# jcfaracco/xpysom-dask

Hardware: AMD Instinct MI355X
Metric: samples/sec/epoch (higher is better)
Workload: dtype f16

## Files before the change

### xpysom_dask_amd/_lib.py

```python
import ctypes as C
import importlib.util
import os

HERE = os.path.dirname(os.path.abspath(__file__))
LIB_PATH = os.environ.get("SOM_LIB_PATH") or os.path.join(HERE, "libsomhip.so")

SOM_DIST = {"euclidean": 0, "euclidean_no_opt": 1, "cosine": 2, "manhattan": 3, "manhattan_no_opt": 3,
            "norm_p": 4, "norm_p_no_opt": 5}
SOM_NEIGH = {"gaussian": 0, "mexican_hat": 1, "bubble": 2, "triangle": 3}
SOM_PREC = {"f32": 0, "bf16": 1, "f16": 3, "exact": 5}
SOM_TOPO = {"rectangular": 0, "hexagonal": 1}
SOM_BMU_ACTIVATION, SOM_BMU_QUANTIZATION = 0, 1
SOM_KERNELS = {"bmu": 0, "segsum": 1, "kron": 2, "merge": 3, "prep": 4, "screen": 5}


class SomConfig(C.Structure):
    _fields_ = [("x", C.c_int32), ("y", C.c_int32), ("input_len", C.c_int32),
                ("distance", C.c_int32), ("neighborhood", C.c_int32),
                ("compact_support", C.c_int32), ("precision", C.c_int32), ("device", C.c_int32),
                ("std_coeff", C.c_double), ("stream", C.c_void_p),
                ("topology", C.c_int32), ("norm_p", C.c_int32), ("norm_p_real", C.c_double)]


_F = C.POINTER(C.c_float)
_I = C.POINTER(C.c_int32)
_H = C.c_void_p

SIGNATURES = {
    "som_version": (C.c_char_p, []),
    "som_device_count": (C.c_int, []),
    "som_last_error": (C.c_char_p, [_H]),
    "som_create": (C.c_int, [C.POINTER(SomConfig), C.POINTER(_H)]),
    "som_destroy": (None, [_H]),
    "som_set_weights": (C.c_int, [_H, _F]),
    "som_get_weights": (C.c_int, [_H, _F]),
    "som_set_data": (C.c_int, [_H, _F, C.c_int64]),
    "som_set_data_device": (C.c_int, [_H, C.c_void_p, C.c_int64]),
    "som_sync_producer": (C.c_int, [_H, C.c_uint64, C.c_int32]),
    "som_copy_to_host": (C.c_int, [_H, C.c_void_p, C.c_uint64, C.c_void_p]),
    "som_epoch_accumulate": (C.c_int, [_H, C.c_double, C.c_double, C.c_int]),
    "som_epoch_accumulate_faithful": (C.c_int, [_H, C.c_double, C.c_double, C.c_int]),
    "som_epoch_merge": (C.c_int, [_H]),
    "som_epoch": (C.c_int, [_H, C.c_double, C.c_double, C.c_int]),
    "som_epoch_accumulate_begin": (C.c_int, [_H, C.c_double, C.c_double, C.c_int]),
    "som_epoch_block_count": (C.c_int, [_H, C.POINTER(C.c_int32)]),
    "som_epoch_accumulate_block": (C.c_int, [_H, C.c_int32, C.POINTER(C.c_int64), C.POINTER(C.c_int64)]),
    "som_comm_load": (C.c_int, [C.c_char_p]),
    "som_comm_unique_id": (C.c_int, [C.c_void_p]),
    "som_comm_init": (C.c_int, [_H, C.c_int32, C.c_int32, C.c_void_p]),
    "som_epoch_allreduce": (C.c_int, [_H]),
    "som_comm_destroy": (C.c_int, [_H]),
    "som_pinned_alloc": (C.c_int, [C.c_uint64, C.POINTER(C.c_void_p)]),
    "som_pinned_free": (C.c_int, [C.c_void_p]),
    "som_stream_begin": (C.c_int, [_H]),
    "som_stream_rows": (C.c_int, [_H, _F, C.c_int64]),
    "som_stream_end": (C.c_int, [_H, C.c_double, C.c_double, C.c_int]),
    "som_accum_device_ptr": (C.c_int, [_H, C.POINTER(C.c_void_p), C.POINTER(C.c_int64)]),
    "som_get_stream": (C.c_int, [_H, C.POINTER(C.c_void_p)]),
    "som_epoch_fetch": (C.c_int, [_H, _F, _F, _I]),
    "som_epoch_accumulate_forced": (C.c_int, [_H, _I, C.c_double, C.c_double, C.c_int]),
    "som_bmu": (C.c_int, [_H, _F, C.c_int64, C.c_int32, _I]),
    "som_bmu_device": (C.c_int, [_H, C.c_void_p, C.c_int64, C.c_int32, _I]),
    "som_bmu_top2": (C.c_int, [_H, _F, C.c_int64, _I, _I]),
    "som_bmu_top2_device": (C.c_int, [_H, C.c_void_p, C.c_int64, _I, _I]),
    "som_bmu_f64": (C.c_int, [_H, C.POINTER(C.c_double), C.c_int64, _I]),
    "som_distance_matrix": (C.c_int, [_H, _F, C.c_int64, C.c_int32, _F]),
    "som_quantization_error": (C.c_int, [_H, _F, C.c_int64, C.POINTER(C.c_double)]),
    "som_quantization_error_device": (C.c_int, [_H, C.c_void_p, C.c_int64, C.POINTER(C.c_double)]),
    "som_set_verify": (C.c_int, [_H, C.c_int32]),
    "som_verify_stats": (C.c_int, [_H, C.POINTER(C.c_int64), C.POINTER(C.c_int64)]),
    "som_debug_corrupt_operands": (C.c_int, [_H, C.c_int32]),
    "som_debug_operand_crc": (C.c_int, [_H, C.c_int32, C.POINTER(C.c_uint64)]),
    "som_debug_exact_centroids": (C.c_int, [_H, C.c_int32, _F, _F, _F, _I]),
    "som_debug_mfma16": (C.c_int, [_H, C.c_void_p, C.c_void_p, _F, _F, C.c_int32]),
    "som_debug_stamps": (C.c_int, [_H, C.c_int64, C.c_void_p]),
    "som_debug_device_bytes": (C.c_int, [C.POINTER(C.c_int64)]),
    "som_debug_qe_stats": (C.c_int, [_H, C.POINTER(C.c_int64), C.POINTER(C.c_int64)]),
    "som_debug_exact_chain_stats": (C.c_int, [_H, C.POINTER(C.c_int64)]),
    "som_debug_exact_select_stats": (C.c_int, [_H, C.POINTER(C.c_int64), C.POINTER(C.c_int64), C.POINTER(C.c_int64)]),
    "som_debug_exact_plan_stats": (C.c_int, [_H, C.POINTER(C.c_int64), C.POINTER(C.c_int64)]),
    "som_debug_exact_last_plan": (C.c_int, [_H, C.POINTER(C.c_int32)]),
    "som_policy_eval": (C.c_int, [C.c_int32, C.POINTER(C.c_double), C.POINTER(C.c_double), C.POINTER(C.c_int32)]),
    "som_policy_replay": (C.c_int, [C.c_int32, C.POINTER(C.c_double), C.POINTER(C.c_double)]),
    "som_operands_replay": (C.c_int, [_I, C.c_int32, _I, _I]),
    "som_patch_order": (C.c_int, [C.c_int32, C.c_int32, _I]),
    "som_exact_stats": (C.c_int, [_H, C.POINTER(C.c_int64), C.POINTER(C.c_int64), C.POINTER(C.c_int64)]),
    "som_exact_top2_stats": (C.c_int, [_H, C.POINTER(C.c_int64), C.POINTER(C.c_int64)]),
    "som_exact_skip_stats": (C.c_int, [_H, C.POINTER(C.c_int64), C.POINTER(C.c_int64)]),
    "som_exact_resident_stats": (C.c_int, [_H, C.POINTER(C.c_int64), C.POINTER(C.c_int64)]),
    "som_exact_scout_stats": (C.c_int, [_H, C.POINTER(C.c_int64), C.POINTER(C.c_int64)]),
    "som_exact_refine_stats": (C.c_int, [_H, C.POINTER(C.c_int64), C.POINTER(C.c_int64)]),
    "som_exact_last_counts": (C.c_int, [_H, _I, C.c_int64]),
    "som_sync": (C.c_int, [_H]),
    "som_profile_enable": (C.c_int, [_H, C.c_int32]),
    "som_profile_get": (C.c_int, [_H, C.c_int32, C.POINTER(C.c_double), C.POINTER(C.c_int64)]),
    "som_profile_reset": (C.c_int, [_H]),
}

_lib = None


def torch_lib_file(name):
    try:
        spec = importlib.util.find_spec("torch")
    except (ImportError, ValueError):
        spec = None
    if spec is None or not spec.submodule_search_locations:
        return None
    cand = os.path.join(list(spec.submodule_search_locations)[0], "lib", name)
    return cand if os.path.exists(cand) else None


def _preload_torch_hip_runtime():
    try:
        spec = importlib.util.find_spec("torch")
    except (ImportError, ValueError):
        spec = None
    if spec is None or not spec.submodule_search_locations:
        return
    cand = os.path.join(list(spec.submodule_search_locations)[0], "lib", "libamdhip64.so")
    if os.path.exists(cand):
        try:
            C.CDLL(cand, mode=C.RTLD_GLOBAL)
        except OSError:
            pass


def load():
    global _lib
    if _lib is not None:
        return _lib
    if not os.path.exists(LIB_PATH):
        raise ImportError(
            f"{LIB_PATH} is missing: build it with `python -m xpysom_dask_amd.build` "
            "(needs hipcc; there is no CPU fallback)")
    if not os.environ.get("SOM_LIB_PATH"):
        from . import build as _build
        have, want = _build.built_hash(LIB_PATH), _build.source_hash()
        if have != want:
            raise ImportError(
                f"{LIB_PATH} is stale: built from sources {have}, the tree is {want}; "
                "rebuild with `python -m xpysom_dask_amd.build`")
    _preload_torch_hip_runtime()
    lib = C.CDLL(LIB_PATH)
    for name, (res, args) in SIGNATURES.items():
        fn = getattr(lib, name)
        fn.restype = res
        fn.argtypes = args
    _lib = lib
    return lib
```

### xpysom_dask_amd/csrc/exact_host.hpp

```cpp

struct PassCtr {
    int* base; int n_groups; bool whole_lines;
    int* gcount() const { return base; }
    int* gstart() const { return base + n_groups; }
    PassCounters* tail() const { return (PassCounters*)(gstart() + n_groups); }
    RowNeed* row_need() const { return (RowNeed*)base; }
    size_t bytes() const {
        const size_t b = 2 * (size_t)n_groups * sizeof(int) + sizeof(PassCounters);
        return whole_lines ? (size_t)round_up((long)b, 64) : b;
    }
};
constexpr size_t EX_CTR_TAIL_INTS = (sizeof(PassCounters) + 64) / sizeof(int);
inline PassCtr pass_ctr(const som_handle* h) { return PassCtr{h->ex.ctr, (int)cdiv(h->K, EX_GROUP), h->ex.chain}; }

constexpr double EX_KAPPA = 6.0;
ExactBound exact_bound(const som_handle* h) {
    const double u = std::ldexp(1.0, -24);
    const double Dl = h->wide ? 32.0 * h->ft_kchunks : 8.0 * h->fr_kg;
    const double n_mfma = h->wide ? h->n_kchunks : h->ks32;
    const double gamma = Dl * u / (1.0 - Dl * u);
    const double slop = 1.01;
    ExactBound eb{};
    eb.cB = (float)(slop * 2.0 * (EX_KAPPA * n_mfma + 1.0) * std::ldexp(1.0, -23));
    eb.cM = (float)(slop * 2.0);
// ... 244 lines not shown
    ex.tile_counts.reset(); ex.tlist.reset(); ex.tcnt.reset(); ex.scout_g.reset(); ex.items.reset(); ex.tile_ticket.reset();
    ex.sk_stride = 0;
    const long tiles = stride / SK_TILE;
    if (int rc = ex.sk_keys.alloc(h, (size_t)stride)) return rc;
    if (int rc = ex.sk_keys2.alloc(h, (size_t)stride)) return rc;
    if (int rc = ex.sk_vals.alloc(h, (size_t)stride)) return rc;
    if (int rc = ex.scout_g.alloc(h, (size_t)stride)) return rc;
    if (h->wide)
        if (int rc = ex.tq.alloc(h, (size_t)stride)) return rc;
    if (int rc = ex.need.alloc(h, (size_t)tiles * ex.cen[0].n_cstages)) return rc;
    if (int rc = ex.need2.alloc(h, (size_t)tiles * ex.cen[1].n_cstages)) return rc;
    if (int rc = ex.glist.alloc(h, (size_t)tiles * n_groups)) return rc;
    if (int rc = ex.gcnt.alloc(h, (size_t)tiles)) return rc;
    if (int rc = ex.tile_counts.alloc(h, (size_t)tiles)) return rc;
    if (int rc = ex.tlist.alloc(h, (size_t)tiles * n_groups * K16_T)) return rc;
    if (int rc = ex.tcnt.alloc(h, (size_t)tiles)) return rc;
    if (int rc = ex.tile_ticket.alloc(h, (size_t)tiles)) return rc;
    ex.item_slots = (int)resident_slots(h, 8);
    if (int rc = ex.items.alloc(h, (size_t)(5 * tiles + 4 * ex.item_slots + 16))) return rc;
    if (int rc = ex.sk_tmp.alloc(h, radix_scratch_ints(stride))) return rc;
    ex.sk_stride = stride;
    return 0;
}

template <class E>
int exact_skip_centroids(som_handle* h, const float* xmax2, unsigned q_blocks, unsigned long long* best64, long n_rows, bool* q_done) {
    auto& ex = h->ex;
    const float* Wsrc = h->ex_patch ? h->Wp : h->W;
    const int n_groups = (int)cdiv(h->K, EX_GROUP);
    auto& c0 = ex.cen[0];
    auto& c1 = ex.cen[1];
    const CentroidLevel l1{c0.Cc, c0.rg, c0.csq, c0.cmax2, c0.n_slots}, l2{c1.Cc, c1.rg, c1.csq, c1.cmax2, c1.n_slots};
    if (!h->ops.centroids_fresh())
        exact_centroids_kernel<<<dim3((unsigned)(cdiv(n_groups, 4) * 4)), dim3(512), 0, h->stream>>>(Wsrc, h->K, h->D, n_groups, l1, l2, h->wmax2);
    const int nst2 = ex.lp.level2 ? c1.n_cstages : 0;
    char* plain = ex.lp.scout ? c0.Cst_plain : nullptr;
    const dim3 tgrid((unsigned)cdiv((long)(c0.n_cstages + nst2) * K16_T, 4)), block(256);
    bool cm = false;
    if (h->ops.take_pending_image(&cm)) {
        const float* Wex = h->ex_patch ? h->Wp : h->W;
        float* cm1 = cm ? (float*)c0.cmax2 : nullptr;
        float* cm2 = cm ? (float*)c1.cmax2 : nullptr;
        const unsigned w_blocks = (unsigned)cdiv((long)h->n_stages * K16_T, 4);
        switch (h->ks32) {
#define SOM_PIMG_CASE(k) case k: exact_prep_images_kernel<k, E><<<dim3(w_blocks + tgrid.x + q_blocks), block, 0, h->stream>>>(w_blocks, tgrid.x, Wex, h->K, h->D, h->Wst, h->n_stages, \
            h->wmax2 + 1, h->Wst_lo, cm1, cm2, l1, c0.Cst, c0.n_cstages, l2, c1.Cst, nst2, xmax2, h->wmax2, plain, h->wn, h->stage_units, best64, n_rows); break;
        SOM_PIMG_CASE(1) SOM_PIMG_CASE(2) SOM_PIMG_CASE(3) SOM_PIMG_CASE(4)
#undef SOM_PIMG_CASE
        default: return fail(h, "exact: block skipping supports input_len <= 128");
        }
        HIPCHK(h, hipGetLastError());
        *q_done = q_blocks > 0;
        return 0;
    }
    switch (h->ks32) {
#define SOM_CIMG_CASE(k) case k: exact_centroid_image_kernel<k, E><<<tgrid, block, 0, h->stream>>>(l1, c0.Cst, c0.n_cstages, l2, c1.Cst, nst2, h->D, xmax2, h->wmax2, plain); break;
    SOM_CIMG_CASE(1) SOM_CIMG_CASE(2) SOM_CIMG_CASE(3) SOM_CIMG_CASE(4)
#undef SOM_CIMG_CASE
    default: return fail(h, "exact: block skipping supports input_len <= 128");
    }
    HIPCHK(h, hipGetLastError());
    return 0;
}

int exact_skip_sortkeys(som_handle* h, som_handle::ExactScratch::SortedRows& sr, long s0, long n, const int* prev, const int* scout_g) {
    auto& ex = h->ex;
    const int n_groups = (int)cdiv(h->K, EX_GROUP);
    if (scout_g != nullptr)
        exact_groupkey_kernel<<<dim3((unsigned)cdiv(n, 256)), dim3(256), 0, h->stream>>>(scout_g, n, n_groups, ex.sk_keys, ex.sk_vals);
    else
        exact_sortkey_kernel<<<dim3((unsigned)cdiv(n, 256)), dim3(256), 0, h->stream>>>(prev, h->ex_inv, n, h->K, ex.sk_keys, ex.sk_vals);
    int bits = 1;
    while ((1L << bits) < n_groups) ++bits;
    return radix_sort_rows(h, ex.sk_keys, n, bits, ex.sk_keys2, sr.order + s0, ex.sk_tmp);
}
template <class E>
int exact_skip_gather(som_handle* h, som_handle::ExactScratch::SortedRows& sr, long s0, const int* order, const float* X, const __bf16* Xb, long n,
                      const float* xsq, const float* xerr, const float* xmax2) {
    const long np = round_up(n, SK_TILE);
    exact_gather_sorted_kernel<E><<<dim3((unsigned)cdiv(np, 16)), dim3(256), 0, h->stream>>>(
        order, n, np, h->dp, h->D, Xb, X, xsq, xerr, xmax2, sr.Xb_s + s0 * h->dp, sr.Xl_s != nullptr ? sr.Xl_s + s0 * h->dp : nullptr, sr.Xf_s + s0 * h->D,
        sr.xsq_s + s0, sr.xerr_s + s0);
    HIPCHK(h, hipGetLastError());
    return 0;
}

template <int KS32, class E>
int exact_scout_nearest_ks(som_handle* h, const __bf16* Xb, long n, unsigned long long* best64, int* g_out) {
    auto& ex = h->ex;
    const auto& c0 = ex.cen[0];
    const void* kern = (const void*)bmu_bf16_k16_kernel<KS32, E, false, false>;
    const size_t lds = 2 * (size_t)k16_stage_bytes(KS32);
    int per_cu = 1;
    if (int rc = kernel_per_cu(h, kern, 64 * K16_NW, lds, &per_cu)) return rc;
    const long blocks = cdiv(n, K16_WG_SAMPLES);
    const long slots = resident_slots(h, per_cu);
    const int parts = std::max(1, std::min(choose_parts(h, blocks, slots, c0.n_cstages), c0.n_cstages));
    bmu_bf16_k16_kernel<KS32, E, false, false><<<dim3((unsigned)blocks, (unsigned)parts), dim3(64 * K16_NW), lds, h->stream>>>(
        Xb, n, c0.Cst_plain, c0.n_cstages, c0.n_slots, best64);
    bmu_finalize_kernel<<<dim3((unsigned)cdiv(n, 256)), dim3(256), 0, h->stream>>>(best64, n, c0.n_slots, g_out);
    HIPCHK(h, hipMemsetAsync(best64, 0xFF, (size_t)n * sizeof(unsigned long long), h->stream));
    HIPCHK(h, hipGetLastError());
    return 0;
}
template <class E>
int exact_scout_nearest(som_handle* h, const __bf16* Xb, long n, unsigned long long* best64, int* g_out) {
    SOM_KS32_DISPATCH(exact_scout_nearest_ks, h, Xb, n, best64, g_out)
    return fail(h, "exact: the scout supports input_len <= 128");
}

template <int KS32, class E>
int exact_scout_pick_ks(som_handle* h, som_handle::ExactScratch::SortedRows& sr, long s0, long n, const int* keys, unsigned long long* best64) {
    auto& ex = h->ex;
    const int n_groups = (int)cdiv(h->K, EX_GROUP);
    const long tiles = round_up(n, SK_TILE) / SK_TILE;
    const size_t lds_l = (size_t)cdiv(n_groups, 64) * sizeof(unsigned long long);
    exact_scout_lists_kernel<<<dim3((unsigned)tiles), dim3(64), lds_l, h->stream>>>(keys, nullptr, n, n_groups, ex.tlist, ex.tcnt);
    const void* kern = (const void*)bmu_bf16_k16_kernel<KS32, E, false, true>;
    const size_t lds = 2 * (size_t)k16_stage_bytes(KS32);
    int per_cu = 1;
    if (int rc = kernel_per_cu(h, kern, 64 * K16_NW, lds, &per_cu)) return rc;
    bmu_bf16_k16_kernel<KS32, E, false, true><<<dim3((unsigned)tiles, 1), dim3(64 * K16_NW), lds, h->stream>>>(
        sr.Xb_s + s0 * h->dp, n, h->Wst, h->n_stages, h->K, best64, nullptr, 0, nullptr, nullptr, nullptr, nullptr, nullptr, nullptr, ExactBound(),
        nullptr, ex.tlist, ex.tcnt);
    exact_scout_pos_kernel<<<dim3((unsigned)cdiv(n, 256)), dim3(256), 0, h->stream>>>(best64, n, h->K, sr.lastpos_s + s0);
    HIPCHK(h, hipGetLastError());
    return 0;
}
template <class E>
int exact_scout_pick(som_handle* h, som_handle::ExactScratch::SortedRows& sr, long s0, long n, const int* keys, unsigned long long* best64) {
    SOM_KS32_DISPATCH(exact_scout_pick_ks, h, sr, s0, n, keys, best64)
    return fail(h, "exact: the scout supports input_len <= 128");
}

void exact_plan_lists(som_handle* h, long tiles, int n_cstages, const unsigned long long* need2) {
    auto& ex = h->ex;
    const int n_groups = (int)cdiv(h->K, EX_GROUP);
    PassCounters* const ctr = pass_ctr(h).tail();
    const int slots = ex.item_queue ? (ex.screen_slots > 0 ? ex.screen_slots : ex.item_slots) : 0;
    int2* const queue = ex.item_queue ? ex.items + 8 : nullptr;
    int* const n_items = (int*)ex.items.p;
    if (ex.chain) {
        exact_lists_totals_kernel<<<dim3((unsigned)cdiv(tiles, LISTS_WG_TILES)), dim3(64 * LISTS_WG_TILES), 0, h->stream>>>(
            ex.need, n_cstages, need2, n_groups, ex.glist, ex.gcnt, ex.tile_counts, ex.tlist, ex.tcnt, tiles, &ctr->lists_done,
            &ctr->blocks_run, &ctr->groups_run, slots, queue, n_items, n_items + 1, ex.item_len_pct, ex.tile_ticket);
        return;
    }
    exact_lists_kernel<<<dim3((unsigned)tiles), dim3(64), 0, h->stream>>>(ex.need, n_cstages, need2, n_groups, ex.glist, ex.gcnt,
                                                                         ex.tile_counts, ex.tlist, ex.tcnt, ex.tile_ticket);
    exact_list_totals_kernel<<<dim3(1), dim3(1024), 0, h->stream>>>(ex.tile_counts, tiles, &ctr->blocks_run, &ctr->groups_run, slots, queue,
                                                                  n_items, n_items + 1, ex.item_len_pct);
}

template <int KS32, class E> constexpr bool plan_fused_fits() { return !(KS32 == 4 && std::is_same<E, Bf16>::value); }
template <class E>
int exact_skip_plan(som_handle* h, som_handle::ExactScratch::SortedRows& sr, long s0, long n, const float* xmax2, const ExactBound& eb,
                    const int* lastpos2, bool time_l2 = false) {
    auto& ex = h->ex;
    PassCounters* const ctr = pass_ctr(h).tail();
    const long np = round_up(n, SK_TILE);
    const long tiles = np / SK_TILE;
    const dim3 block(64 * K16_NW);
    const auto& c0 = ex.cen[0];
    const auto& c1 = ex.cen[1];
    const long want = (1024 + tiles - 1) / tiles;
    const long parts_cap = ex.hook_plan_parts > 0 ? ex.hook_plan_parts : 4L;
    const dim3 pgrid((unsigned)tiles, (unsigned)std::max<long>(1, std::min<long>({want, parts_cap, (long)c0.n_cstages})));
    const size_t lds1 = 2 * (size_t)h->stage_bytes + (size_t)c0.n_cstages * 8;
    const size_t lds2 = 2 * (size_t)h->stage_bytes + (size_t)c0.n_cstages * 64 * sizeof(int) + (size_t)c1.n_cstages * 8;
    const bool l2 = ex.lp.level2;
    const int force = ex.skip_mode == 3 ? 1 : 0;
    const __bf16* Xs = sr.Xb_s + s0 * h->dp;
    const size_t lds = lds2 + (size_t)c0.n_cstages * 8 + (size_t)SK_TILE * sizeof(float);
    const bool fits = h->ks32 != 4 || plan_fused_fits<4, E>();
    if (ex.fuse_plan && ex.chain && l2 && lastpos2 == nullptr && pgrid.y == 1 && !time_l2 && lds <= 160 * 1024 && fits) {
        PlanListsOut lo;
        lo.n_groups = (int)cdiv(h->K, EX_GROUP);
        lo.glist = ex.glist; lo.gcnt = ex.gcnt; lo.tile_counts = ex.tile_counts; lo.tlist = ex.tlist; lo.tcnt = ex.tcnt;
        lo.tile_ticket = ex.tile_ticket;
        lo.done = &ctr->lists_done; lo.blocks_run = &ctr->blocks_run; lo.groups_run = &ctr->groups_run;
        lo.slots = ex.item_queue ? (ex.screen_slots > 0 ? ex.screen_slots : ex.item_slots) : 0;
        lo.items = ex.item_queue ? ex.items + 8 : nullptr;
        lo.n_items = (int*)ex.items.p; lo.item_ctr = lo.n_items + 1; lo.len_pct = ex.item_len_pct;
#define SOM_PLAN_FUSED_CASE(k) case k: if constexpr (plan_fused_fits<k, E>()) { \
        { int pc; if (int rc = kernel_per_cu(h, (const void*)exact_plan_fused_kernel<k, E>, 64 * K16_NW, lds, &pc)) return rc; } \
        exact_plan_fused_kernel<k, E><<<dim3((unsigned)tiles), block, lds, h->stream>>>(Xs, n, c0.Cst, c0.n_cstages, c0.cmax2, c1.Cst, c1.n_slots, \
            c1.cmax2, sr.xsq_s + s0, sr.xerr_s + s0, xmax2, h->wmax2, h->wmax2 + 1, eb, sr.lastpos_s + s0, h->Wst, sr.seed_s + s0, force, lo); \
        } break;
        switch (h->ks32) {
        SOM_PLAN_FUSED_CASE(1) SOM_PLAN_FUSED_CASE(2) SOM_PLAN_FUSED_CASE(3) SOM_PLAN_FUSED_CASE(4)
        default: return fail(h, "exact: block skipping supports input_len <= 128");
        }
#undef SOM_PLAN_FUSED_CASE
        ++ex.plan_fused_launches;
        HIPCHK(h, hipGetLastError());
        return 0;
    }
    ++ex.plan_split_launches;
    unsigned long long* const need2_clear = l2 && ex.chain ? ex.need2.p : nullptr;
    if (l2 && !ex.chain) HIPCHK(h, hipMemsetAsync(ex.need2, 0, (size_t)tiles * c1.n_cstages * sizeof(unsigned long long), h->stream));
#define SOM_PLAN_CASE(k) case k: { \
        { int pc; if (int rc = kernel_per_cu(h, (const void*)exact_plan_kernel<k, E, false>, 64 * K16_NW, lds1, &pc)) return rc; } \
        exact_plan_kernel<k, E, false><<<pgrid, block, lds1, h->stream>>>(Xs, n, c0.Cst, c0.n_cstages, c0.rg, c0.n_slots, \
            sr.xsq_s + s0, sr.xerr_s + s0, sr.sU_s + s0, xmax2, c0.cmax2, h->wmax2, h->wmax2 + 1, eb, ex.need, sr.lastpos_s + s0, \
            h->Wst, sr.seed_s + s0, nullptr, 0, force, lastpos2, lastpos2 != nullptr ? &ctr->scout_wins : nullptr, need2_clear); \
        if (l2) { \
            if (time_l2) (void)hipEventRecord(ex.cost.ev[3], h->stream); \
            { int pc; if (int rc = kernel_per_cu(h, (const void*)exact_plan_kernel<k, E, true>, 64 * K16_NW, lds2, &pc)) return rc; } \
            exact_plan_kernel<k, E, true><<<dim3((unsigned)tiles, pgrid.y), block, lds2, h->stream>>>(Xs, n, c1.Cst, c1.n_cstages, c1.rg, c1.n_slots, \
                sr.xsq_s + s0, sr.xerr_s + s0, sr.sU_s + s0, xmax2, c1.cmax2, h->wmax2, h->wmax2 + 1, eb, ex.need2, nullptr, \
                nullptr, nullptr, ex.need, c0.n_cstages, force); \
            if (time_l2) (void)hipEventRecord(ex.cost.ev[4], h->stream); \
        } } break;
    switch (h->ks32) {
    SOM_PLAN_CASE(1) SOM_PLAN_CASE(2) SOM_PLAN_CASE(3) SOM_PLAN_CASE(4)
    default: return fail(h, "exact: block skipping supports input_len <= 128");
    }
#undef SOM_PLAN_CASE
    exact_plan_lists(h, tiles, c0.n_cstages, l2 ? ex.need2.p : nullptr);
    HIPCHK(h, hipGetLastError());
    return 0;
}

template <class E>
int exact_wide_centroids(som_handle* h, const float* xmax2) {
    auto& ex = h->ex;
    auto& c0 = ex.cen[0];
    const float* Wsrc = h->ex_patch ? h->Wp : h->W;
    const int n_groups = (int)cdiv(h->K, EX_GROUP);
    wide_centroids_kernel<<<dim3((unsigned)n_groups), dim3(256), 0, h->stream>>>(Wsrc, h->K, h->D, n_groups, c0.Cc, c0.rg, c0.csq, c0.cmax2, h->wmax2);
    const long total = (long)c0.n_img_stages * WD_T * h->n_kchunks * 64;
    prep_w_bf16_wide_kernel<E><<<dim3((unsigned)cdiv(total, 256)), dim3(256), 0, h->stream>>>(c0.Cc, n_groups, h->D, h->n_kchunks, c0.Cst, c0.n_img_stages,
                                                                                             nullptr, h->wmax2);
    exact_werr_kernel<E><<<dim3((unsigned)cdiv(n_groups, 4 * EX_WERR_UNITS)), dim3(256), 0, h->stream>>>(c0.Cc, n_groups, h->D, h->wmax2, c0.cmax2 + 1, nullptr);
    char* plain = ex.lp.scout ? c0.Cst_plain : nullptr;
    if (plain) HIPCHK(h, hipMemcpyAsync(plain, c0.Cst, (size_t)c0.n_img_stages * h->stage_bytes, hipMemcpyDeviceToDevice, h->stream));
    wide_centroid_tail_kernel<<<dim3((unsigned)cdiv((long)c0.n_img_stages * WD_STAGE_UNITS, 256)), dim3(256), 0, h->stream>>>(
        c0.rg, c0.csq, n_groups, c0.Cst, c0.n_img_stages, h->stage_bytes, xmax2, h->wmax2, plain);
    HIPCHK(h, hipGetLastError());
    return 0;
}

template <class E>
int exact_wide_gather(som_handle* h, som_handle::ExactScratch::SortedRows& sr, long s0, const float* X, long n, const float* xsq, const float* xerr,
                      const int* prev, const float* xmax2) {
    const long np = round_up(n, SK_TILE);
    wide_gather_sorted_kernel<<<dim3((unsigned)cdiv(np, 4)), dim3(256), 0, h->stream>>>(sr.order + s0, n, np, h->D, X, xsq, xerr, prev,
                                                                                      sr.Xf_s + s0 * h->D, sr.xsq_s + s0, sr.xerr_s + s0, sr.lastpos_s + s0);
    const long n_blocks = np / h->tl_bm;
    const long total = n_blocks * h->n_kchunks * (h->tl_bm / 16) * TL_KS * 64;
    prep_tiles_bf16_kernel<E><<<dim3((unsigned)cdiv(total, 256)), dim3(256), 0, h->stream>>>(
        sr.Xf_s + s0 * h->D, n, h->D, h->n_kchunks, n_blocks, h->tl_bm, h->tl_xtile, 1.0f, nullptr, (char*)(sr.Xb_s + s0 * h->dp), xmax2);
    HIPCHK(h, hipGetLastError());
    return 0;
}

template <int KS32, class E>
int exact_wide_scout_nearest_ks(som_handle* h, const __bf16* Ximg, long n, unsigned long long* best64, int* g_out) {
    auto& ex = h->ex;
    const auto& c0 = ex.cen[0];
    const size_t lds = (size_t)WD_SLOTS * wd_stage_bytes(KS32);
    int per_cu = 1;
    if (int rc = kernel_per_cu(h, (const void*)bmu_bf16_wide_kernel<KS32, E>, 64 * WD_NW, lds, &per_cu)) return rc;
    const long blocks = cdiv(n, WD_WG_SAMPLES);
    const long slots = resident_slots(h, per_cu);
    const int parts = (int)std::max<long>(1, std::min<long>({cdiv(2 * slots, blocks), 8L, (long)c0.n_img_stages}));
    bmu_bf16_wide_kernel<KS32, E><<<dim3((unsigned)blocks, (unsigned)parts), dim3(64 * WD_NW), lds, h->stream>>>(
        (const char*)Ximg, n, c0.Cst_plain, c0.n_img_stages, best64);
    bmu_finalize_kernel<<<dim3((unsigned)cdiv(n, 256)), dim3(256), 0, h->stream>>>(best64, n, c0.n_slots, g_out);
    HIPCHK(h, hipMemsetAsync(best64, 0xFF, (size_t)n * sizeof(unsigned long long), h->stream));
    HIPCHK(h, hipGetLastError());
    return 0;
}
template <int KS32, class E>
int exact_wide_scout_pick_ks(som_handle* h, som_handle::ExactScratch::SortedRows& sr, long s0, long n, const int* keys, unsigned long long* best64) {
    auto& ex = h->ex;
    const int n_groups = (int)cdiv(h->K, EX_GROUP);
    const long tiles = round_up(n, SK_TILE) / SK_TILE;
    const size_t lds_l = (size_t)cdiv(n_groups, 64) * sizeof(unsigned long long);
    exact_scout_lists_kernel<<<dim3((unsigned)tiles), dim3(64), lds_l, h->stream>>>(keys, nullptr, n, n_groups, ex.glist, ex.gcnt, 1);
    const size_t lds = (size_t)WD_SLOTS * wd_stage_bytes(KS32);
    int per_cu = 1;
    if (int rc = kernel_per_cu(h, (const void*)bmu_bf16_wide_kernel<KS32, E, false, true>, 64 * WD_NW, lds, &per_cu)) return rc;
    bmu_bf16_wide_kernel<KS32, E, false, true><<<dim3((unsigned)tiles, 1), dim3(64 * WD_NW), lds, h->stream>>>(
        (const char*)(sr.Xb_s + s0 * h->dp), n, h->Wst, h->n_stages, best64, nullptr, 0, nullptr, nullptr, nullptr, nullptr, nullptr, nullptr, ExactBound(),
        ex.glist, ex.gcnt, n_groups);
    exact_scout_pos_kernel<<<dim3((unsigned)cdiv(n, 256)), dim3(256), 0, h->stream>>>(best64, n, h->K, sr.lastpos_s + s0, h->ex_perm);
    HIPCHK(h, hipGetLastError());
    return 0;
}
template <class E>
int exact_wide_scout_nearest(som_handle* h, const __bf16* Ximg, long n, unsigned long long* best64, int* g_out) {
    SOM_WIDE_DISPATCH(exact_wide_scout_nearest_ks, h, Ximg, n, best64, g_out)
    return fail(h, "exact: no wide scout instance for this input_len");
}
template <class E>
int exact_wide_scout_pick(som_handle* h, som_handle::ExactScratch::SortedRows& sr, long s0, long n, const int* keys, unsigned long long* best64) {
    SOM_WIDE_DISPATCH(exact_wide_scout_pick_ks, h, sr, s0, n, keys, best64)
    return fail(h, "exact: no wide scout instance for this input_len");
}

template <int KS32, class E>
int exact_wide_plan_ks(som_handle* h, som_handle::ExactScratch::SortedRows& sr, long s0, long n, const float* xmax2, const ExactBound& eb) {
    auto& ex = h->ex;
    const auto& c0 = ex.cen[0];
    const long np = round_up(n, SK_TILE);
    const long tiles = np / SK_TILE;
    exact_seed_kernel<<<dim3((unsigned)cdiv(n * 16, 256)), dim3(256), 0, h->stream>>>(
        sr.Xf_s + s0 * h->D, n, h->D, h->W, h->wsq, h->K, sr.lastpos_s + s0, sr.xsq_s + s0, sr.xerr_s + s0, h->wmax2, xmax2, h->wmax2 + 1, eb, ex.seed, ex.tq);
    wide_plan_rows_kernel<<<dim3((unsigned)cdiv(n, 256)), dim3(256), 0, h->stream>>>(n, sr.xsq_s + s0, sr.xerr_s + s0, ex.tq, xmax2, c0.cmax2, h->wmax2,
                                                                                  h->wmax2 + 1, eb, ex.skip_mode == 3 ? 1 : 0, sr.seed_s + s0, sr.sU_s + s0);
    HIPCHK(h, hipMemsetAsync(ex.need, 0, (size_t)tiles * c0.n_cstages * sizeof(unsigned long long), h->stream));
    auto kern = bmu_bf16_wide_kernel<KS32, E, false, false, true>;
    const size_t lds = (size_t)WD_SLOTS * wd_stage_bytes(KS32) + (size_t)c0.n_cstages * sizeof(unsigned long long);
    int per_cu = 1;
    if (int rc = kernel_per_cu(h, (const void*)kern, 64 * WD_NW, lds, &per_cu)) return rc;
    const long slots = resident_slots(h, per_cu);
    int parts = (int)std::max<long>(1, std::min<long>({cdiv(2 * slots, tiles), 8L, (long)c0.n_img_stages}));
    bmu_bf16_wide_kernel<KS32, E, false, false, true><<<dim3((unsigned)tiles, (unsigned)parts), dim3(64 * WD_NW), lds, h->stream>>>(
        (const char*)(sr.Xb_s + s0 * h->dp), n, c0.Cst, c0.n_img_stages, nullptr, nullptr, 0, nullptr, nullptr, nullptr, nullptr, nullptr, nullptr, ExactBound(),
        nullptr, nullptr, 0, sr.seed_s + s0, sr.sU_s + s0, ex.need, c0.n_cstages);
    exact_plan_lists(h, tiles, c0.n_cstages, nullptr);
    HIPCHK(h, hipGetLastError());
    return 0;
}
template <class E>
int exact_wide_plan(som_handle* h, som_handle::ExactScratch::SortedRows& sr, long s0, long n, const float* xmax2, const ExactBound& eb) {
    SOM_WIDE_DISPATCH(exact_wide_plan_ks, h, sr, s0, n, xmax2, eb)
    return fail(h, "exact: no wide plan instance for this input_len");
}

template <int KG>
int exact_rescore_kg(som_handle* h, const float* X, unsigned long long* best64, int deint) {
    auto& ex = h->ex;
    auto kern = exact_rescore_mfma_kernel<KG>;
    const size_t lds = (size_t)fr_stage_bytes(KG);
    int per_cu = 1;
    if (int rc = kernel_per_cu(h, (const void*)kern, 256, lds, &per_cu)) return rc;
    const long grid = std::min<long>(ex.max_tiles, h->ex.grid_mult * resident_slots(h, per_cu));
    kern<<<dim3((unsigned)grid), dim3(256), lds, h->stream>>>(X, h->D, h->Wfst, h->K, ex.tile_tab, &pass_ctr(h).tail()->n_tiles, ex.plist,
                                                             best64, h->ex_perm, nullptr, h->ex_sub44 ? 1 : 0, deint, nullptr);
    return 0;
}

inline unsigned exact_tiles_blocks(const som_handle* h) { return h->ex.chain ? 16u : 1u; }

template <int KS32, class E>
int exact_refine_ks(som_handle* h, som_handle::ExactScratch::SortedRows& sr, long r0, long n, const float* xmax2, const ExactBound& eb) {
    auto& ex = h->ex;
    const PassCtr pc = pass_ctr(h);
    const int n_groups = pc.n_groups;
    int* gcount = pc.gcount(); PassCounters* const ctr = pc.tail();
    int* n_tiles = &ctr->n_tiles;
    exact_tiles_kernel<<<dim3(exact_tiles_blocks(h)), dim3(1024), 0, h->stream>>>(gcount, n_groups, ex.stride, ex.stride * ex.pairs, ex.tile_tab, n_tiles,
                                                                                 &ctr->overflow, nullptr, nullptr, &ctr->pairs_in);
    uint32_t* rowmin2 = (uint32_t*)ex.rowarg.p;
    if (!ex.chain) HIPCHK(h, hipMemsetAsync(rowmin2, 0xFF, (size_t)n * sizeof(uint32_t), h->stream));
    const size_t lds = (size_t)k16_stage_bytes(KS32) + (size_t)K16_T * KS32 * 1024;
    int per_cu = 1;
    if (int rc = kernel_per_cu(h, (const void*)exact_refine_kernel<KS32, E>, 256, lds, &per_cu)) return rc;
    const long grid = std::min<long>(ex.max_tiles, h->ex.grid_mult * resident_slots(h, per_cu));
    exact_refine_kernel<KS32, E><<<dim3((unsigned)grid), dim3(256), lds, h->stream>>>(
        sr.Xb_s + r0 * h->dp, sr.Xl_s + r0 * h->dp, h->Wst, h->Wst_lo, ex.tile_tab, n_tiles, ex.plist, ex.gmin, rowmin2);
    exact_thr2_kernel<<<dim3((unsigned)cdiv(n, 256)), dim3(256), 0, h->stream>>>(rowmin2, n, sr.xsq_s + r0, sr.xerr_s + r0, h->wmax2, xmax2,
                                                                               h->wmax2 + 1, eb);
    exact_select2_kernel<<<dim3((unsigned)n_groups), dim3(256), 0, h->stream>>>(ex.plist, ex.gmin, ex.stride, gcount, rowmin2, &ctr->pairs_out);
    HIPCHK(h, hipGetLastError());
    return 0;
}
template <class E>
int exact_refine(som_handle* h, som_handle::ExactScratch::SortedRows& sr, long r0, long n, const float* xmax2, const ExactBound& eb) {
// ... 365 lines not shown
```

### xpysom_dask_amd/csrc/exact_skip.hpp

```cpp
#pragma once
#include "bmu_bf16_k16.hpp"
#include "bmu_f32_res.hpp"

namespace somhip {

constexpr int SK_TILE = K16_WG_SAMPLES;
static_assert(K16_STAGE_UNITS == 64 && K16_T == 4, "block skipping: a stage of the resident screen is one 64-unit group of four 16-unit tiles");

struct CentroidLevel { float* C; float* rg; float* csq; float* cmax2; int n_slots; };
struct CentroidShared {
    float qsum[4][128];
    float part[2][64][2];
    float csq_s[2][5];
};
__device__ __forceinline__ void group_centroids(const float (&w)[16], int g, int K, int D, const CentroidLevel& l1,
                                                const CentroidLevel& l2, CentroidShared& sh) {
    const int tid = threadIdx.x, lane = tid & 63;
    const int d = tid & 127, q = tid >> 7, fh = (tid >> 6) & 1;
    const int cnt = (int)max(0L, min(64L, (long)K - (long)g * 64));
    const int cb = max(0, min(16, cnt - 16 * q));
    float sum = 0.0f;
#pragma unroll
    for (int k = 0; k < 16; ++k) sum += w[k];
    sh.qsum[q][d] = sum;
// ... 67 lines not shown
    __shared__ int u_s[64];
    __shared__ float den_s[64];
    const int g = blockIdx.x, tid = threadIdx.x;
    const int d = tid & 127, q = tid >> 7;
    const int cnt = (int)max(0L, min(64L, (long)K - (long)g * 64));
    const int cb = max(0, min(16, cnt - 16 * q));
    if (tid < cnt) {
        const int pos = g * 64 + tid;
        const int u = o.perm != nullptr ? o.perm[pos] : pos;
        u_s[tid] = u;
        den_s[tid] = ACC[(long)u * D1p + D];
    }
    __syncthreads();
    float w[16];
#pragma unroll
    for (int k = 0; k < 16; ++k) {
        const bool on = d < D && k < cb;
        const long u = on ? u_s[16 * q + k] : 0;
        const float* src = !on ? ACC : den_s[16 * q + k] != 0.0f ? ACC + u * D1p + d : o.W + u * D + d;
        const float v = *src;
        w[k] = on ? v : 0.0f;
    }
#pragma unroll
    for (int k = 0; k < 16; ++k) {
        const bool on = d < D && k < cb;
        const int i = 16 * q + k;
        const float den = on ? den_s[i] : 0.0f;
        const float v = w[k] / den;
        w[k] = den != 0.0f ? v : w[k];
        if (on) {
            const long u = u_s[i];
            if (den != 0.0f) o.W[u * D + d] = w[k];
            if (o.Wp != nullptr) o.Wp[((long)g * 64 + i) * D + d] = w[k];
            ws[i * MPX_STRIDE + d] = w[k];
        }
    }
    if (l1.C != nullptr && g == 0 && tid == 0) { l1.cmax2[1] = 0.0f; l2.cmax2[1] = 0.0f; }
    if (l1.C != nullptr) group_centroids(w, g, K, D, l1, l2, sh);
    else __syncthreads();
    if (g >= n_groups) return;
    if (o.Wfst != nullptr) {
        char* base = o.Wfst + (long)g * fr_stage_bytes(o.fr_kg);
        for (int r = tid; r < FR_UT * o.fr_kg * 64; r += 512) {
            const int lane = r & 63, t = r >> 6;
            const int gk = t % o.fr_kg, i = (t / o.fr_kg) * 32 + (lane & 31);
            f32x4 v;
#pragma unroll
            for (int j = 0; j < 4; ++j) {
                const int k = 8 * gk + 2 * j + (lane >> 5);
                v[j] = (i < cnt && k < D) ? ws[i * MPX_STRIDE + k] : 0.0f;
            }
            *(f32x4*)(base + (long)r * 16) = v;
        }
    }
    if (tid < 64) {
        float qv = __builtin_inff(), m = 0.0f;
        if (tid < cnt) {
            const int pos = g * 64 + tid;
            qv = np_pairwise_sq_sum_leaf((const float*)(ws + tid * MPX_STRIDE), D);
            o.wsq[u_s[tid]] = qv;
            if (o.wsq_p != nullptr) o.wsq_p[pos] = qv;
            o.wn[pos] = qv;
            m = (qv == qv) ? qv : 0.0f;
        }
        if (o.Wfst != nullptr) ((float*)(o.Wfst + (long)g * fr_stage_bytes(o.fr_kg) + (long)FR_UT * o.fr_kg * 1024))[tid] = qv;
#pragma unroll
        for (int s = 32; s > 0; s >>= 1) m = fmaxf(m, __shfl_xor(m, s, 64));
        if (tid == 0) atomic_max_pos_f32(o.wmax2, m);
    }
}

__global__ __launch_bounds__(256) void exact_sortkey_kernel(const int* __restrict__ prev, const int* __restrict__ inv, long n,
                                                            int K, int* __restrict__ keys, int* __restrict__ vals) {
    const long i = (long)blockIdx.x * 256 + threadIdx.x;
    if (i >= n) return;
    int u = prev[i];
    u = u < 0 ? 0 : u >= K ? K - 1 : u;
    keys[i] = (inv != nullptr ? inv[u] : u) >> 6;
    vals[i] = (int)i;
}

__global__ __launch_bounds__(256) void exact_lastpos_kernel(const int* __restrict__ prev, const int* __restrict__ order,
                                                            const int* __restrict__ inv, long n, int K, int* __restrict__ lastpos) {
    const long p = (long)blockIdx.x * 256 + threadIdx.x;
    if (p >= n) return;
    int u = prev[order[p]];
    u = u < 0 ? 0 : u >= K ? K - 1 : u;
    lastpos[p] = inv != nullptr ? inv[u] : u;
}

template <class EL>
__global__ __launch_bounds__(256) void exact_gather_sorted_kernel(const int* __restrict__ order, long n, long np, int dp, int D,
                                                                  const __bf16* __restrict__ Xb, const float* __restrict__ X,
                                                                  const float* __restrict__ xsq, const float* __restrict__ xerr,
                                                                  const float* __restrict__ xmax2,
                                                                  __bf16* __restrict__ Xb_s, __bf16* __restrict__ Xl_s,
                                                                  float* __restrict__ Xf_s,
                                                                  float* __restrict__ xsq_s, float* __restrict__ xerr_s) {
    using E = typename EL::T;
    using bf16x8 = typename V8<E>::t;
    const int lane = threadIdx.x & 15;
    const long p = (long)blockIdx.x * 16 + (threadIdx.x >> 4);
    if (p >= np) return;
    const long r = p < n ? (long)order[p] : -1;
    const float sx = ex_scale(*xmax2);
    const bool vec = (D & 7) == 0;
    for (int c = lane; c < dp / 8; c += 16) {
        bf16x8 v, vl;
#pragma unroll
        for (int j = 0; j < 8; ++j) { v[j] = (E)0.0f; vl[j] = (E)0.0f; }
        if (r >= 0) {
            v = *(const bf16x8*)((const char*)Xb + (r * dp + c * 8) * 2);
            float f[8];
            if (vec && c * 8 < D) {
                const f32x4 a = *(const f32x4*)(X + r * D + c * 8), b = *(const f32x4*)(X + r * D + c * 8 + 4);
                const f32x4 ev = {a[0], a[2], b[0], b[2]}, od = {a[1], a[3], b[1], b[3]};
                *(f32x4*)(Xf_s + p * D + c * 4) = ev;
                *(f32x4*)(Xf_s + p * D + D / 2 + c * 4) = od;
#pragma unroll
                for (int j = 0; j < 4; ++j) { f[j] = a[j]; f[4 + j] = b[j]; }
            } else {
#pragma unroll
                for (int j = 0; j < 8; ++j) {
                    f[j] = c * 8 + j < D ? X[r * D + c * 8 + j] : 0.0f;
                    if (c * 8 + j < D) Xf_s[p * D + c * 8 + j] = f[j];
                }
            }
#pragma unroll
            for (int j = 0; j < 8; ++j) {
                const float d = (f[j] * sx - (float)v[j]) * 2048.0f;
                vl[j] = cvt<E>(d == d && __builtin_fabsf(d) < 3.0e38f ? d : 0.0f);
            }
        }
        *(bf16x8*)((char*)Xb_s + (p * dp + c * 8) * 2) = v;
        if (Xl_s != nullptr) *(bf16x8*)((char*)Xl_s + (p * dp + c * 8) * 2) = vl;
    }
    if (lane == 0) {
        const float nanv = __builtin_nanf("");
        xsq_s[p] = r >= 0 ? xsq[r] : nanv;
        xerr_s[p] = r >= 0 ? xerr[r] : nanv;
    }
}

__device__ __forceinline__ float up_to_half(float v) {
    if (!(v == v)) return v;
    if (v > 65504.0f) return __builtin_inff();
    if (v < 0x1p-14f) return 0x1p-14f;
    const _Float16 hv = (_Float16)v;
    float f = (float)hv;
    if (f < v) f = (float)__builtin_bit_cast(_Float16, (unsigned short)(__builtin_bit_cast(unsigned short, hv) + 1));
    return f;
}

__device__ __forceinline__ uint32_t row16_or(uint32_t v) {
    v |= (uint32_t)__builtin_amdgcn_update_dpp(0, (int)v, 0x121, 0xF, 0xF, false);
    v |= (uint32_t)__builtin_amdgcn_update_dpp(0, (int)v, 0x122, 0xF, 0xF, false);
    v |= (uint32_t)__builtin_amdgcn_update_dpp(0, (int)v, 0x124, 0xF, 0xF, false);
    v |= (uint32_t)__builtin_amdgcn_update_dpp(0, (int)v, 0x128, 0xF, 0xF, false);
    return v;
}

template <int KS32, class EL>
__device__ __forceinline__ void exact_centroid_image_body(const unsigned bid, const CentroidLevel& l1, char* __restrict__ Cst1, int n_cstages1,
                                                          const CentroidLevel& l2, char* __restrict__ Cst2, int n_cstages2, int D,
                                                          const float* __restrict__ xmax2, const float* __restrict__ wmax2,
                                                          char* __restrict__ Cst1_plain) {
    using E = typename EL::T;
    using bf16x8 = typename V8<E>::t;
    constexpr int STAGE = k16_stage_bytes(KS32);
    const int lane = threadIdx.x & 63;
    long tile = (long)bid * 4 + (threadIdx.x >> 6);
    const long t1 = (long)n_cstages1 * K16_T;
    const bool second = tile >= t1;
    if (second) tile -= t1;
    if (tile >= (long)(second ? n_cstages2 : n_cstages1) * K16_T) return;
    const CentroidLevel& lv = second ? l2 : l1;
    char* Cst = second ? Cst2 : Cst1;
    const long stage = tile / K16_T;
    const int t16 = (int)(tile - stage * K16_T);
    const long slot = stage * K16_STAGE_UNITS + t16 * 16 + (lane & 15);
    const float sw = ex_scale(*wmax2), sx = ex_scale(*xmax2);
    float er = 0.0f;
#pragma unroll
    for (int ks = 0; ks < KS32; ++ks) {
        const int k0 = ks * 32 + (lane >> 4) * 8;
        bf16x8 v;
#pragma unroll
        for (int j = 0; j < 8; ++j) {
            const float f = (slot < lv.n_slots && k0 + j < D) ? lv.C[slot * D + k0 + j] * sw : 0.0f;
            const E hb = cvt<E>(-f);
            v[j] = hb;
            const float e = half_operand_error(-f, (float)hb);
            er = __builtin_fmaf(e, e, er);
        }
        *(bf16x8*)(Cst + stage * STAGE + ((long)(t16 * KS32 + ks) * 64 + lane) * 16) = v;
        if (!second && Cst1_plain != nullptr) *(bf16x8*)(Cst1_plain + stage * STAGE + ((long)(t16 * KS32 + ks) * 64 + lane) * 16) = v;
    }
    er += __shfl_xor(er, 16, 64);
    er += __shfl_xor(er, 32, 64);
    float m = (er == er) ? er : 0.0f;
#pragma unroll
    for (int o = 8; o > 0; o >>= 1) m = fmaxf(m, __shfl_xor(m, o, 64));
    if (lane == 0) atomic_max_pos_f32(lv.cmax2 + 1, m);
    if (lane < 16) {
        float* tail = (float*)(Cst + (stage + 1) * (long)STAGE - 1024);
        const int within = t16 * 16 + lane;
        const float rad = slot < lv.n_slots ? lv.rg[slot] : -1.0f;
        float* ptail = (!second && Cst1_plain != nullptr) ? (float*)(Cst1_plain + (stage + 1) * (long)STAGE - 1024) : nullptr;
        if (rad < 0.0f) { tail[within] = __builtin_inff(); tail[64 + within] = 0.0f; if (ptail) ptail[within] = __builtin_inff(); }
        else {
            const float big = __builtin_sqrtf(*wmax2) * __builtin_sqrtf(*xmax2) * (1.0f + 1.0f / 1024.0f);
            const float S = sx * sw, hS = 0.5f * S * (1.0f + 1.0f / 1024.0f);
            const float s0 = __builtin_fmaf(0.5f * S, lv.csq[slot], S * big);
            tail[within] = s0 - hS * rad * rad * (1.0f + 0x1p-20f);
            tail[64 + within] = -up_to_half(sw * rad);
            if (ptail) ptail[within] = (s0 == s0 && s0 < 3.0e38f) ? s0 : __builtin_inff();
        }
    }
}
template <int KS32, class EL>
__global__ __launch_bounds__(256) void exact_centroid_image_kernel(CentroidLevel l1, char* __restrict__ Cst1, int n_cstages1,
                                                                   CentroidLevel l2, char* __restrict__ Cst2, int n_cstages2, int D,
                                                                   const float* __restrict__ xmax2, const float* __restrict__ wmax2,
                                                                   char* __restrict__ Cst1_plain = nullptr) {
    exact_centroid_image_body<KS32, EL>(blockIdx.x, l1, Cst1, n_cstages1, l2, Cst2, n_cstages2, D, xmax2, wmax2, Cst1_plain);
}

template <int KS32, class EL>
__global__ __launch_bounds__(256) void exact_prep_images_kernel(unsigned w_blocks, unsigned c_blocks, const float* __restrict__ W, int K, int D,
                                                                char* __restrict__ Wst, int n_stages, float* __restrict__ werr2,
                                                                char* __restrict__ Wst_lo, float* __restrict__ cm1, float* __restrict__ cm2,
                                                                CentroidLevel l1, char* __restrict__ Cst1, int n_cstages1,
                                                                CentroidLevel l2, char* __restrict__ Cst2, int n_cstages2,
                                                                const float* __restrict__ xmax2, const float* __restrict__ wmax2,
                                                                char* __restrict__ Cst1_plain, const float* __restrict__ wn,
                                                                int stage_units, unsigned long long* __restrict__ best64, long n_rows) {
    if (blockIdx.x < w_blocks) prep_w_exact_k16_body<KS32, EL>(blockIdx.x, W, K, D, Wst, n_stages, wmax2, werr2, Wst_lo, cm1, cm2, false);
    else if (blockIdx.x < w_blocks + c_blocks)
        exact_centroid_image_body<KS32, EL>(blockIdx.x - w_blocks, l1, Cst1, n_cstages1, l2, Cst2, n_cstages2, D, xmax2, wmax2, Cst1_plain);
    else prep_wsqh_body(blockIdx.x - w_blocks - c_blocks, wn, K, wmax2, xmax2, Wst, n_stages, k16_stage_bytes(KS32), stage_units, best64, n_rows, 1);
}

template <int KS32, class EL>
__device__ __forceinline__ float plan_row_seed(const typename V8<typename EL::T>::t (&xrow)[KS32], long row, float q, float xe,
                                               const ExactBound& eb, const ExactScales& sw, const char* __restrict__ Wst,
                                               const int* __restrict__ lastpos, const int* __restrict__ lastpos2,
                                               int* __restrict__ scout_wins, float* __restrict__ seed_s, int force_all) {
    using bf16x8 = typename V8<typename EL::T>::t;
    constexpr int STAGE = k16_stage_bytes(KS32);
    const int lane = threadIdx.x & 63, quad = lane >> 4;
    auto value_of = [&](int pos) -> float {
        const char* stg = Wst + (long)(pos >> 6) * STAGE;
        const int t16 = (pos >> 4) & 3, c = pos & 15;
        float d = 0.0f;
#pragma unroll
        for (int ks = 0; ks < KS32; ++ks) {
            const bf16x8 a = *(const bf16x8*)(stg + ((t16 * KS32 + ks) * 64 + quad * 16 + c) * 16);
#pragma unroll
            for (int jj = 0; jj < 8; ++jj) d = __builtin_fmaf((float)a[jj], (float)xrow[ks][jj], d);
        }
        d += __shfl_xor(d, 16, 64);
        d += __shfl_xor(d, 32, 64);
        return *(const float*)(stg + K16_T * KS32 * 1024 + (t16 * 16 + c) * 4) + d;
    };
    float vu = value_of(lastpos[row]);
    if (lastpos2 != nullptr) {
        const float v2 = value_of(lastpos2[row]);
        const float Sq = sw.sx * sw.sw;
        const float ua = q + 2.0f * (vu / Sq - sw.big), ub = q + 2.0f * (v2 / Sq - sw.big);
        const bool win = ua < 0.9f * ub;
        const unsigned long long wm = __ballot(win && quad == 0);
        if (scout_wins != nullptr && lane == __builtin_ctzll(__ballot(true)) && wm != 0ull) atomicAdd(scout_wins, (int)__popcll(wm));
        vu = (v2 < vu || !(vu == vu)) ? v2 : vu;
    }
    const float Sw = sw.sx * sw.sw;
    const float e = ex_row_bound(eb, sw, q, xe);
    const float f32s = ex_f32_share(eb, sw, q);
    const float e_valu = 48.0f * 0x1p-24f * Sw * sw.bmag;
    const float sd = vu + (e - f32s) * (1.0f + 1.0f / 1024.0f) + e_valu + Sw * sw.bmag * 0x1p-21f;
    if (quad == 0) seed_s[row] = (sd > 0.0f && sd < 3.0e38f) ? sd : __builtin_inff();
    const float e_one = 0.5f * (e - f32s) * (1.0f + 1.0f / 1024.0f) + e_valu;
    const float tau_up = 2.0f * (((vu + e_one) - Sw * sw.big) / Sw) + 0x1p-20f * (sw.big + __builtin_fabsf(vu) / Sw);
    const float xn = __builtin_sqrtf(q) * (1.0f + 1.0f / 1024.0f);
    const float share = 2.0f * (eb.cA * xn * sw.wm + eb.cW * sw.wm * sw.wm);
    const float U0 = q * (1.0f + 1.0f / 1024.0f) + tau_up + share * (1.0f + 1.0f / 1024.0f) + 0x1p-18f * (q + __builtin_fabsf(tau_up));
    const float U = U0 < 0.0f ? 0.0f : U0;
    float su = __builtin_sqrtf(U) * (1.0f + 1.0f / 1024.0f);
    if (force_all || !(su == su) || !(su < 3.0e38f) || !(e == e)) su = __builtin_inff();
    return su;
}

template <int KS32>
__device__ __forceinline__ void plan_row_threshold(const ExactBound& eb, const ExactScales& sc, bool in_pass, float q, float xe, float su,
                                                   float& P, float& bx) {
    const float S = sc.sx * sc.sw;
    float A = -__builtin_inff(), sU = 0.0f;
    if (in_pass) {
        const float ec = 0.5f * ex_row_bound(eb, sc, q, xe) * (1.0f + 1.0f / 1024.0f);
        sU = su;
        A = S * sc.big + ec - 0.5f * S * q * (1.0f - 1.0f / 1024.0f) + 0x1p-12f * S * (sc.big + q) + 0x1p-16f * S * sc.wm * sc.wm;
        if (!(A == A) || !(A < 3.0e38f) || !(su < 3.0e38f)) {
            A = __builtin_inff(); sU = 0.0f;
        }
    }
    bx = up_to_half(sc.sx * sU * (1.0f + 1.0f / 1024.0f));
    P = A + 0.5f * S * (1.0f + 1.0f / 1024.0f) * sU * sU * (1.0f + 0x1p-20f) + (float)(24 * (KS32 + 1)) * 0x1p-23f * S * sc.bmag;
    if (!(bx < 3.0e38f) || !(P == P)) P = __builtin_inff();
    if (A == -__builtin_inff()) P = -__builtin_inff();
}
template <class EL>
__device__ __forceinline__ typename V8<typename EL::T>::t plan_extra_step(float bx) {
    using E = typename EL::T;
    typename V8<E>::t v;
#pragma unroll
    for (int jj = 0; jj < 8; ++jj) v[jj] = (E)0.0f;
    if (((threadIdx.x & 63) >> 4) == 0 && bx < 3.0e38f) v[0] = (E)bx;
    return v;
}

template <int KS32, class EL>
__device__ __forceinline__ void plan_run_tile(int j, const typename V8<typename EL::T>::t (&a)[KS32], const f32x4& wv, float rneg,
                                              const typename V8<typename EL::T>::t (&xf)[K16_SB][KS32],
                                              const typename V8<typename EL::T>::t (&xe)[K16_SB], const float (&P)[K16_SB],
                                              uint32_t& lane_bits) {
    using E = typename EL::T;
    using bf16x8 = typename V8<E>::t;
    bf16x8 ae;
#pragma unroll
    for (int jj = 0; jj < 8; ++jj) ae[jj] = (E)0.0f;
    if (((threadIdx.x & 63) >> 4) == 0) ae[0] = (E)rneg;
    f32x4 acc[K16_SB];
#pragma unroll
    for (int sb = 0; sb < K16_SB; ++sb) acc[sb] = wv;
#pragma unroll
    for (int ks = 0; ks < KS32; ++ks)
#pragma unroll
        for (int sb = 0; sb < K16_SB; ++sb) acc[sb] = mfma16(a[ks], xf[sb][ks], acc[sb]);
#pragma unroll
    for (int sb = 0; sb < K16_SB; ++sb) acc[sb] = mfma16(ae, xe[sb], acc[sb]);
#pragma unroll
    for (int r = 0; r < 4; ++r) {
        bool nd = false;
#pragma unroll
        for (int sb = 0; sb < K16_SB; ++sb) nd = nd || !(acc[sb][r] > P[sb]);
        lane_bits |= nd ? (1u << (4 * j + r)) : 0u;
    }
}
template <int KS32, class EL>
__device__ __forceinline__ void plan_load_tile(const char* st, int t, typename V8<typename EL::T>::t (&a)[KS32], f32x4& wv, float& rneg) {
    using bf16x8 = typename V8<typename EL::T>::t;
    const int lane = threadIdx.x & 63;
    const float* wq = (const float*)(st + K16_T * KS32 * 1024);
#pragma unroll
    for (int ks = 0; ks < KS32; ++ks) a[ks] = *(const bf16x8*)(st + ((t * KS32 + ks) * 64 + lane) * 16);
    wv = *(const f32x4*)(wq + t * 16 + 4 * (lane >> 4));
    rneg = wq[64 + t * 16 + (lane & 15)];
}

template <int KS32, class EL>
__device__ __forceinline__ void plan_walk_level1(const char* __restrict__ Cst, int s_begin, int s_end, char* smem, unsigned long long* nl,
                                                 const typename V8<typename EL::T>::t (&xf)[K16_SB][KS32],
                                                 const typename V8<typename EL::T>::t (&xe)[K16_SB], const float (&P)[K16_SB]) {
    using bf16x8 = typename V8<typename EL::T>::t;
    constexpr int STAGE = k16_stage_bytes(KS32);
    constexpr int PIECES = K16_T * KS32 + 1;
    const int lane = threadIdx.x & 63, quad = lane >> 4, col = lane & 15;
    const int wave = __builtin_amdgcn_readfirstlane(threadIdx.x >> 6);
    auto dma_stage = [&](int s, char* dst) {
        const char* src = Cst + (long)s * STAGE;
        for (int p = wave; p < PIECES; p += K16_NW) lds_dma_16(src + (long)p * 1024 + lane * 16, dst + p * 1024);
    };
    if (s_begin < s_end) dma_stage(s_begin, smem);
    for (int i = s_begin; i < s_end; ++i) {
        asm volatile("s_waitcnt vmcnt(0) lgkmcnt(0)" ::: "memory");
        __builtin_amdgcn_s_barrier();
        asm volatile("" ::: "memory");
        if (i + 1 < s_end) dma_stage(i + 1, smem + ((i + 1 - s_begin) & 1) * STAGE);
        const char* st = smem + ((i - s_begin) & 1) * STAGE;
        uint32_t lane_bits = 0u;
        bf16x8 aA[KS32], aB[KS32];
        f32x4 wvA, wvB;
        float rnA, rnB;
        plan_load_tile<KS32, EL>(st, 0, aA, wvA, rnA);
        plan_load_tile<KS32, EL>(st, 1, aB, wvB, rnB);
        plan_run_tile<KS32, EL>(0, aA, wvA, rnA, xf, xe, P, lane_bits);
        plan_load_tile<KS32, EL>(st, 2, aA, wvA, rnA);
        plan_run_tile<KS32, EL>(1, aB, wvB, rnB, xf, xe, P, lane_bits);
        plan_load_tile<KS32, EL>(st, 3, aB, wvB, rnB);
        plan_run_tile<KS32, EL>(2, aA, wvA, rnA, xf, xe, P, lane_bits);
        plan_run_tile<KS32, EL>(3, aB, wvB, rnB, xf, xe, P, lane_bits);
        const uint32_t any_row = row16_or(lane_bits);
        if (col == 0 && any_row != 0u) {
            const uint32_t lo = ((any_row & 15u) | (((any_row >> 4) & 15u) << 16)) << (4 * quad);
            const uint32_t hi = (((any_row >> 8) & 15u) | (((any_row >> 12) & 15u) << 16)) << (4 * quad);
            atomicOr(nl + (i - s_begin), ((unsigned long long)hi << 32) | lo);
        }
    }
}

__device__ __forceinline__ void plan_level2_list(const unsigned long long* need1, int n_cstages1, int n_slots2, int* act, int* act_n) {
    const int lane = threadIdx.x & 63;
    int cnt = 0;
    for (int s1 = 0; s1 < n_cstages1; ++s1) {
        const unsigned long long w = need1[s1];
        const int g = s1 * 64 + lane;
        const bool on = ((w >> lane) & 1ull) && 4 * (g >> 2) * 4 < n_slots2;
        const unsigned long long mk = __ballot(on);
        if (on) act[cnt + __popcll(mk & ((1ull << lane) - 1ull))] = g;
        cnt += __popcll(mk);
    }
    if (lane == 0) *act_n = cnt;
}

template <int KS32, class EL>
__device__ __forceinline__ void plan_walk_level2(const char* __restrict__ Cst, const int* act, int b0, int e0, char* smem,
                                                 unsigned long long* nl, const typename V8<typename EL::T>::t (&xf)[K16_SB][KS32],
                                                 const typename V8<typename EL::T>::t (&xe)[K16_SB], const float (&P)[K16_SB]) {
    using bf16x8 = typename V8<typename EL::T>::t;
    constexpr int STAGE = k16_stage_bytes(KS32);
    static_assert(K16_NW == 4, "a wave per tile fills the slot's tail");
    const int lane = threadIdx.x & 63, quad = lane >> 4, col = lane & 15;
    const int wave = __builtin_amdgcn_readfirstlane(threadIdx.x >> 6);
    constexpr int TQ = K16_T * KS32 * 1024;
    auto frag_of = [&](int g, int sub, int ks, int q) -> const char* {
        return Cst + (long)(g >> 4) * STAGE + (((((g >> 2) & 3) * KS32 + ks) * 64 + q * 16 + 4 * (g & 3) + sub) * 16);
    };
    auto dma_chunk = [&](int c0, char* dst) {
        for (int p = wave; p < K16_T * KS32; p += K16_NW) {
            const int j = p / KS32, ks = p - j * KS32;
            if (c0 + 4 * j < e0) {
                const int gi = c0 + 4 * j + (col >> 2);
                const int g = gi < e0 ? act[gi] : act[c0 + 4 * j];
                lds_dma_16(frag_of(g, col & 3, ks, quad), dst + p * 1024);
            }
        }
    };
    auto load_tail = [&](int c0) -> float {
        const int i = lane & 15, gi = c0 + 4 * wave + (i >> 2);
        if (lane >= 32 || gi >= e0) return lane < 16 ? __builtin_inff() : 0.0f;
        const int g = act[gi];
        return *(const float*)(Cst + (long)(g >> 4) * STAGE + TQ + (((lane >> 4) * 64) + ((g >> 2) & 3) * 16 + 4 * (g & 3) + (i & 3)) * 4);
    };
    auto store_tail = [&](char* dst, float v) {
        if (lane < 32) *(float*)(dst + TQ + (((lane >> 4) * 64) + wave * 16 + (lane & 15)) * 4) = v;
    };
    if (b0 < e0) { dma_chunk(b0, smem); store_tail(smem, load_tail(b0)); }
    int k = 0;
    for (int c0 = b0; c0 < e0; c0 += 16, ++k) {
        asm volatile("s_waitcnt vmcnt(0) lgkmcnt(0)" ::: "memory");
        __builtin_amdgcn_s_barrier();
        asm volatile("" ::: "memory");
        char* sn = smem + ((k + 1) & 1) * STAGE;
        float tail_n = 0.0f;
        if (c0 + 16 < e0) { dma_chunk(c0 + 16, sn); tail_n = load_tail(c0 + 16); }
        const char* st = smem + (k & 1) * STAGE;
        uint32_t lane_bits = 0u;
        bf16x8 aA[KS32], aB[KS32];
        f32x4 wvA, wvB;
        float rnA, rnB;
        const bool h1 = c0 + 4 < e0, h2 = c0 + 8 < e0, h3 = c0 + 12 < e0;
        plan_load_tile<KS32, EL>(st, 0, aA, wvA, rnA);
        if (h1) plan_load_tile<KS32, EL>(st, 1, aB, wvB, rnB);
        plan_run_tile<KS32, EL>(0, aA, wvA, rnA, xf, xe, P, lane_bits);
        if (h1) {
            if (h2) plan_load_tile<KS32, EL>(st, 2, aA, wvA, rnA);
            plan_run_tile<KS32, EL>(1, aB, wvB, rnB, xf, xe, P, lane_bits);
            if (h2) {
                if (h3) plan_load_tile<KS32, EL>(st, 3, aB, wvB, rnB);
                plan_run_tile<KS32, EL>(2, aA, wvA, rnA, xf, xe, P, lane_bits);
                if (h3) plan_run_tile<KS32, EL>(3, aB, wvB, rnB, xf, xe, P, lane_bits);
            }
        }
        const uint32_t any_row = row16_or(lane_bits);
        if (col == 0 && any_row != 0u) {
#pragma unroll
            for (int j = 0; j < 4; ++j) {
                const uint32_t nib = (any_row >> (4 * j)) & 15u;
                const int gi = c0 + 4 * j + quad;
                if (nib != 0u && gi < e0) {
                    const int g = act[gi];
                    atomicOr(nl + (g >> 4), (unsigned long long)nib << (4 * (g & 15)));
                }
            }
        }
        if (c0 + 16 < e0) store_tail(sn, tail_n);
    }
}

template <int KS32, class EL, bool LEVEL2>
__global__ __launch_bounds__(64 * K16_NW, LEVEL2 ? 3 : 2) void exact_plan_kernel(const __bf16* __restrict__ Xb, long N,
                                                                    const char* __restrict__ Cst, int n_cstages,
                                                                    const float* __restrict__ rg, int n_slots,
                                                                    const float* __restrict__ xsq, const float* __restrict__ xerr,
                                                                    float* __restrict__ sU_s,
                                                                    const float* __restrict__ xmax2, const float* __restrict__ cmax2,
                                                                    const float* __restrict__ wmax2, const float* __restrict__ werr2,
                                                                    ExactBound eb, unsigned long long* __restrict__ need,
                                                                    const int* __restrict__ lastpos, const char* __restrict__ Wst,
                                                                    float* __restrict__ seed_s,
                                                                    const unsigned long long* __restrict__ need1, int n_cstages1,
                                                                    int force_all, const int* __restrict__ lastpos2 = nullptr,
                                                                    int* __restrict__ scout_wins = nullptr,
                                                                    unsigned long long* __restrict__ need2_clear = nullptr) {
    using bf16x8 = typename V8<typename EL::T>::t;
    constexpr int DP = 32 * KS32;
    constexpr int STAGE = k16_stage_bytes(KS32);
    extern __shared__ __attribute__((aligned(16))) char smem[];
    __shared__ int act_n;

    const int tid = threadIdx.x, lane = tid & 63;
    const int wave = __builtin_amdgcn_readfirstlane(tid >> 6);
    const int quad = lane >> 4, col = lane & 15;
    const long wave_s0 = (long)blockIdx.x * K16_WG_SAMPLES + wave * (16 * K16_SB);

    bf16x8 xf[K16_SB][KS32];
    bf16x8 xe[K16_SB];
    float P[K16_SB];
    const ExactScales sc = ex_scales(xmax2, cmax2, cmax2 + 1);
    const ExactScales sw = ex_scales(xmax2, wmax2, werr2);
#pragma unroll
    for (int sb = 0; sb < K16_SB; ++sb) {
        const long row = wave_s0 + sb * 16 + col;
#pragma unroll
        for (int ks = 0; ks < KS32; ++ks) xf[sb][ks] = *(const bf16x8*)(Xb + row * DP + ks * 32 + quad * 8);
        float q = 0.0f, xer = 0.0f, su = 0.0f;
        if (row < N) {
            q = xsq[row]; xer = xerr[row];
            if constexpr (!LEVEL2) {
                su = plan_row_seed<KS32, EL>(xf[sb], row, q, xer, eb, sw, Wst, lastpos, lastpos2, scout_wins, seed_s, force_all);
                if (quad == 0) sU_s[row] = su;
            } else {
                su = sU_s[row];
            }
        }
        float bx;
        plan_row_threshold<KS32>(eb, sc, row < N, q, xer, su, P[sb], bx);
        xe[sb] = plan_extra_step<EL>(bx);
    }

    int* act = (int*)(smem + 2 * STAGE);
    unsigned long long* nl = (unsigned long long*)(smem + 2 * STAGE + (LEVEL2 ? (size_t)n_cstages1 * 64 * sizeof(int) : 0));
    for (int i = tid; i < n_cstages; i += 64 * K16_NW) nl[i] = 0ull;
    if constexpr (LEVEL2) {
        if (wave == 0) plan_level2_list(need1 + (long)blockIdx.x * n_cstages1, n_cstages1, n_slots, act, &act_n);
        __syncthreads();
        const int n_act = act_n;
        const int c_all = (n_act + 15) / 16;
        const int b0 = 16 * (int)((long)c_all * blockIdx.y / gridDim.y);
        const int e0 = min(n_act, 16 * (int)((long)c_all * (blockIdx.y + 1) / gridDim.y));
        plan_walk_level2<KS32, EL>(Cst, act, b0, e0, smem, nl, xf, xe, P);
        __syncthreads();
        for (int i = tid; i < n_cstages; i += 64 * K16_NW)
            if (nl[i] != 0ull) atomicOr(need + (long)blockIdx.x * n_cstages + i, nl[i]);
        return;
    }
    const int s_begin = (int)((long)n_cstages * blockIdx.y / gridDim.y);
    const int s_end = (int)((long)n_cstages * (blockIdx.y + 1) / gridDim.y);
    plan_walk_level1<KS32, EL>(Cst, s_begin, s_end, smem, nl, xf, xe, P);
    __syncthreads();
    for (int i = s_begin + tid; i < s_end; i += 64 * K16_NW) need[(long)blockIdx.x * n_cstages + i] = nl[i - s_begin];
    if (need2_clear != nullptr)
        for (int i = 4 * s_begin + tid; i < 4 * s_end; i += 64 * K16_NW) need2_clear[(long)blockIdx.x * 4 * n_cstages + i] = 0ull;
}

template <bool PUBLISH>
__device__ __forceinline__ void exact_lists_tile(const long tile, const int lane, const unsigned long long* __restrict__ need1, int n_cstages,
                                                 const unsigned long long* __restrict__ need2, int n_groups,
                                                 int* __restrict__ glist, int* __restrict__ gcnt,
                                                 int2* tile_counts, int* __restrict__ tlist,
                                                 int* __restrict__ tcnt, int* __restrict__ tile_ticket) {
    const unsigned long long below = (1ull << lane) - 1ull;
    int base = 0, blk = 0, kept = 0;
    for (int s0 = 0; s0 < n_cstages; s0 += 64) {
        const unsigned long long mine = s0 + lane < n_cstages ? need1[s0 + lane] : 0ull;
        const uint32_t lo = (uint32_t)mine, hi = (uint32_t)(mine >> 32);
        unsigned long long todo = __ballot(mine != 0ull);
        for (; todo != 0ull; todo &= todo - 1ull) {
            const int sl = (int)__builtin_ctzll(todo), s = s0 + sl;
            const unsigned long long w = ((unsigned long long)(uint32_t)__builtin_amdgcn_readlane((int)hi, sl) << 32) |
                                         (uint32_t)__builtin_amdgcn_readlane((int)lo, sl);
            uint32_t nib = 15u;
            if (need2 != nullptr) nib = (uint32_t)(need2[4 * s + (lane >> 4)] >> (4 * (lane & 15))) & 15u;
            const int g = s * 64 + lane;
            const bool l1 = ((w >> lane) & 1ull) && g < n_groups;
            const bool on = l1 && nib != 0u;
            const unsigned long long mk = __ballot(on);
            if (on) glist[tile * n_groups + base + __popcll(mk & ((1ull << lane) - 1ull))] = (g << 4) | (int)nib;
            base += __popcll(mk);
            kept += __popcll(__ballot(l1));
            int before = 0, total = 0;
#pragma unroll
            for (int b = 0; b < 4; ++b) {
                const unsigned long long mb = __ballot(on && ((nib >> b) & 1u));
                before += __popcll(mb & below);
                total += __popcll(mb);
            }
            if (on) {
                int o = blk + before;
#pragma unroll
                for (int b = 0; b < 4; ++b)
                    if ((nib >> b) & 1u) tlist[tile * 4 * n_groups + o++] = (g << 2) | b;
            }
            blk += total;
        }
    }
    if (lane == 0) {
        gcnt[tile] = base; tcnt[tile] = blk;
        tile_ticket[tile] = 0;
        if (PUBLISH)
            __hip_atomic_store((unsigned long long*)(tile_counts + tile), ((unsigned long long)(uint32_t)kept << 32) | (uint32_t)blk,
                               __ATOMIC_RELAXED, __HIP_MEMORY_SCOPE_AGENT);
        else tile_counts[tile] = make_int2(blk, kept);
    }
}
__global__ __launch_bounds__(64) void exact_lists_kernel(const unsigned long long* __restrict__ need1, int n_cstages,
                                                         const unsigned long long* __restrict__ need2, int n_groups,
                                                         int* __restrict__ glist, int* __restrict__ gcnt,
                                                         int2* __restrict__ tile_counts, int* __restrict__ tlist,
                                                         int* __restrict__ tcnt, int* __restrict__ tile_ticket) {
    exact_lists_tile<false>(blockIdx.x, threadIdx.x, need1 + (long)blockIdx.x * n_cstages, n_cstages,
                            need2 != nullptr ? need2 + (long)blockIdx.x * 4 * n_cstages : nullptr, n_groups, glist, gcnt, tile_counts, tlist, tcnt, tile_ticket);
}

template <int NT>
__device__ __forceinline__ void exact_list_totals_body(const int2* tile_counts, long tiles, int* __restrict__ blocks_run,
                                                       int* __restrict__ groups_run, int slots, int2* __restrict__ items,
                                                       int* __restrict__ n_items, int* __restrict__ item_ctr, int len_pct,
                                                       int* sb, int* sk, int& tot_b) {
    const int tid = threadIdx.x, lane = tid & 63, wave = tid >> 6;
    int b = 0, k = 0;
    for (long t = tid; t < tiles; t += NT) { const int2 c = tile_counts[t]; b += c.x; k += c.y; }
#pragma unroll
    for (int o = 32; o > 0; o >>= 1) { b += __shfl_xor(b, o, 64); k += __shfl_xor(k, o, 64); }
    if (lane == 0) { sb[wave] = b; sk[wave] = k; }
    __syncthreads();
    if (tid == 0) {
        b = 0; k = 0;
        for (int w = 0; w < NT / 64; ++w) { b += sb[w]; k += sk[w]; }
        *blocks_run = b; *groups_run = k;
        tot_b = b;
    }
    if (items == nullptr) return;
    __syncthreads();
    const long total = tot_b;
    const long by_mean = (len_pct * total) / (100 * (tiles > 0 ? tiles : 1)) + 1, by_slots = total / (2 * (long)(slots > 0 ? slots : 1));
    const int L = (int)max(32L, min(by_mean, by_slots));
    auto parts_of = [&](int cnt) -> int { return cnt <= L ? 1 : (cnt + L - 1) / L; };
    const long per = (tiles + NT - 1) / NT, t_b = min((long)tid * per, tiles), t_e = min(t_b + per, tiles);
    int mine = 0;
    for (long t = t_b; t < t_e; ++t) mine += parts_of(tile_counts[t].x);
    int incl = mine;
#pragma unroll
    for (int o = 1; o < 64; o <<= 1) { const int v = __shfl_up(incl, o, 64); if (lane >= o) incl += v; }
    __syncthreads();
    if (lane == 63) sb[wave] = incl;
    __syncthreads();
    int before = 0, all = 0;
#pragma unroll
    for (int w = 0; w < NT / 64; ++w) { if (w < wave) before += sb[w]; all += sb[w]; }
    int o = before + incl - mine;
    for (long t = t_b; t < t_e; ++t) {
        const int np = parts_of(tile_counts[t].x);
        for (int q = 0; q < np; ++q) items[o++] = make_int2((int)t, q | (np << 16));
    }
    if (tid == 0) { *n_items = all; *item_ctr = 0; }
}
__global__ __launch_bounds__(1024) void exact_list_totals_kernel(const int2* __restrict__ tile_counts, long tiles, int* __restrict__ blocks_run,
                                                                 int* __restrict__ groups_run, int slots = 0, int2* __restrict__ items = nullptr,
                                                                 int* __restrict__ n_items = nullptr, int* __restrict__ item_ctr = nullptr,
                                                                 int len_pct = 125) {
    __shared__ int sb[16], sk[16];
    __shared__ int tot_b;
    exact_list_totals_body<1024>(tile_counts, tiles, blocks_run, groups_run, slots, items, n_items, item_ctr, len_pct, sb, sk, tot_b);
}

constexpr int LISTS_WG_TILES = 16;
__device__ __forceinline__ bool exact_lists_last(int* __restrict__ done, int* last_s) {
    asm volatile("s_waitcnt vmcnt(0)" ::: "memory");
    __syncthreads();
    if (threadIdx.x == 0) {
        const int ticket = __hip_atomic_fetch_add(done, 1, __ATOMIC_RELAXED, __HIP_MEMORY_SCOPE_AGENT);
        *last_s = ticket == (int)gridDim.x - 1 ? 1 : 0;
        if (*last_s) {
            __builtin_amdgcn_fence(__ATOMIC_ACQUIRE, "agent");
            asm volatile("s_waitcnt vmcnt(0)" ::: "memory");
            __hip_atomic_store(done, 0, __ATOMIC_RELAXED, __HIP_MEMORY_SCOPE_AGENT);
        }
    }
    __syncthreads();
    return *last_s != 0;
}
struct PlanListsOut {
    int n_groups;
    int* glist; int* gcnt; int2* tile_counts; int* tlist; int* tcnt; int* tile_ticket;
    int* done; int* blocks_run; int* groups_run;
    int slots; int2* items; int* n_items; int* item_ctr; int len_pct;
};
__global__ __launch_bounds__(64 * LISTS_WG_TILES) void exact_lists_totals_kernel(const unsigned long long* __restrict__ need1, int n_cstages,
                                                                                const unsigned long long* __restrict__ need2, int n_groups,
                                                                                int* __restrict__ glist, int* __restrict__ gcnt,
                                                                                int2* tile_counts, int* __restrict__ tlist,
                                                                                int* __restrict__ tcnt, long tiles, int* __restrict__ done,
                                                                                int* __restrict__ blocks_run, int* __restrict__ groups_run,
                                                                                int slots, int2* __restrict__ items, int* __restrict__ n_items,
                                                                                int* __restrict__ item_ctr, int len_pct,
                                                                                int* __restrict__ tile_ticket) {
    static_assert(LISTS_WG_TILES == 16, "the totals' scan is written for sixteen waves");
    __shared__ int sb[16], sk[16];
    __shared__ int tot_b;
    __shared__ int last;
    const int tid = threadIdx.x;
    const long tile = (long)blockIdx.x * LISTS_WG_TILES + (tid >> 6);
    if (tile < tiles)
        exact_lists_tile<true>(tile, tid & 63, need1 + tile * n_cstages, n_cstages, need2 != nullptr ? need2 + tile * 4 * n_cstages : nullptr, n_groups,
                               glist, gcnt, tile_counts, tlist, tcnt, tile_ticket);
    if (!exact_lists_last(done, &last)) return;
    exact_list_totals_body<64 * LISTS_WG_TILES>(tile_counts, tiles, blocks_run, groups_run, slots, items, n_items, item_ctr, len_pct, sb, sk, tot_b);
}

template <int KS32, class EL>
__global__ __launch_bounds__(64 * K16_NW, 3) void exact_plan_fused_kernel(const __bf16* __restrict__ Xb, long N,
                                                                    const char* __restrict__ Cst1, int n_cstages1, const float* __restrict__ cmax2_1,
                                                                    const char* __restrict__ Cst2, int n_slots2, const float* __restrict__ cmax2_2,
                                                                    const float* __restrict__ xsq, const float* __restrict__ xerr,
                                                                    const float* __restrict__ xmax2,
                                                                    const float* __restrict__ wmax2, const float* __restrict__ werr2,
                                                                    ExactBound eb, const int* __restrict__ lastpos, const char* __restrict__ Wst,
                                                                    float* __restrict__ seed_s, int force_all, PlanListsOut lo) {
    using bf16x8 = typename V8<typename EL::T>::t;
    constexpr int DP = 32 * KS32;
    constexpr int STAGE = k16_stage_bytes(KS32);
    constexpr int NT = 64 * K16_NW;
    extern __shared__ __attribute__((aligned(16))) char smem[];
    __shared__ int act_n;
    __shared__ int sb_s[NT / 64], sk_s[NT / 64];
    __shared__ int tot_b;
    __shared__ int last;

    const int tid = threadIdx.x, lane = tid & 63;
    const int wave = __builtin_amdgcn_readfirstlane(tid >> 6);
    const int quad = lane >> 4, col = lane & 15;
    const long wave_s0 = (long)blockIdx.x * K16_WG_SAMPLES + wave * (16 * K16_SB);
    const int n_cstages2 = 4 * n_cstages1;
    int* act = (int*)(smem + 2 * STAGE);
    unsigned long long* nl2 = (unsigned long long*)(smem + 2 * STAGE + (size_t)n_cstages1 * 64 * sizeof(int));
    unsigned long long* nl1 = nl2 + n_cstages2;
    float* p2s = (float*)(nl1 + n_cstages1);

    bf16x8 xf[K16_SB][KS32];
    bf16x8 xe[K16_SB];
    float P[K16_SB];
    {
        const ExactScales sc1 = ex_scales(xmax2, cmax2_1, cmax2_1 + 1);
        const ExactScales sc2 = ex_scales(xmax2, cmax2_2, cmax2_2 + 1);
        const ExactScales sw = ex_scales(xmax2, wmax2, werr2);
#pragma unroll
        for (int sb = 0; sb < K16_SB; ++sb) {
            const long row = wave_s0 + sb * 16 + col;
#pragma unroll
            for (int ks = 0; ks < KS32; ++ks) xf[sb][ks] = *(const bf16x8*)(Xb + row * DP + ks * 32 + quad * 8);
            float q = 0.0f, xer = 0.0f, su = 0.0f;
            if (row < N) {
                q = xsq[row]; xer = xerr[row];
                su = plan_row_seed<KS32, EL>(xf[sb], row, q, xer, eb, sw, Wst, lastpos, nullptr, nullptr, seed_s, force_all);
            }
            float bx1, bx2, P2;
            plan_row_threshold<KS32>(eb, sc1, row < N, q, xer, su, P[sb], bx1);
            plan_row_threshold<KS32>(eb, sc2, row < N, q, xer, su, P2, bx2);
            xe[sb] = plan_extra_step<EL>(P[sb] == __builtin_inff() ? bx2 : bx1);
            if (quad == 0) p2s[wave * (16 * K16_SB) + sb * 16 + col] = P2;
        }
    }
    for (int i = tid; i < n_cstages1 + n_cstages2; i += NT) nl2[i] = 0ull;

    plan_walk_level1<KS32, EL>(Cst1, 0, n_cstages1, smem, nl1, xf, xe, P);
    __syncthreads();
    if (wave == 0) plan_level2_list(nl1, n_cstages1, n_slots2, act, &act_n);
#pragma unroll
    for (int sb = 0; sb < K16_SB; ++sb) P[sb] = p2s[wave * (16 * K16_SB) + sb * 16 + col];
    __syncthreads();
    plan_walk_level2<KS32, EL>(Cst2, act, 0, act_n, smem, nl2, xf, xe, P);
    __syncthreads();
    if (wave == 0)
        exact_lists_tile<true>(blockIdx.x, lane, nl1, n_cstages1, nl2, lo.n_groups, lo.glist, lo.gcnt, lo.tile_counts, lo.tlist, lo.tcnt, lo.tile_ticket);
    if (!exact_lists_last(lo.done, &last)) return;
    exact_list_totals_body<NT>(lo.tile_counts, gridDim.x, lo.blocks_run, lo.groups_run, lo.slots, lo.items, lo.n_items, lo.item_ctr, lo.len_pct,
                               sb_s, sk_s, tot_b);
}

__global__ __launch_bounds__(256) void exact_groupkey_kernel(const int* __restrict__ g, long n, int n_groups, int* __restrict__ keys,
                                                             int* __restrict__ vals) {
    const long i = (long)blockIdx.x * 256 + threadIdx.x;
    if (i >= n) return;
    const int v = g[i];
    keys[i] = v < 0 ? 0 : v >= n_groups ? n_groups - 1 : v;
    vals[i] = (int)i;
}

__global__ __launch_bounds__(64) void exact_scout_lists_kernel(const int* __restrict__ gkey, const int* __restrict__ lastpos, long n,
                                                               int n_groups, int* __restrict__ tlist, int* __restrict__ tcnt,
                                                               int group_items = 0) {
    extern __shared__ unsigned long long sbm[];
    const long tile = blockIdx.x;
    const int lane = threadIdx.x;
    const int nw = (n_groups + 63) / 64;
    for (int w = lane; w < nw; w += 64) sbm[w] = 0ull;
    __syncthreads();
    for (int i = 0; i < SK_TILE / 64; ++i) {
        const long p = tile * SK_TILE + i * 64 + lane;
        if (p < n) {
            int g = gkey[p];
            g = g < 0 ? 0 : g >= n_groups ? n_groups - 1 : g;
            atomicOr(sbm + (g >> 6), 1ull << (g & 63));
            if (lastpos != nullptr) {
                int g2 = lastpos[p] >> 6;
                g2 = g2 < 0 ? 0 : g2 >= n_groups ? n_groups - 1 : g2;
                atomicOr(sbm + (g2 >> 6), 1ull << (g2 & 63));
            }
        }
    }
    __syncthreads();
    int base = 0;
    int* out = tlist + tile * (group_items ? 1 : 4) * (long)n_groups;
    for (int w0 = 0; w0 < nw; w0 += 64) {
        unsigned long long word = w0 + lane < nw ? sbm[w0 + lane] : 0ull;
        const int c = __popcll(word);
        int incl = c;
#pragma unroll
        for (int o = 1; o < 64; o <<= 1) { const int t = __shfl_up(incl, o, 64); if (lane >= o) incl += t; }
        int at = base + incl - c;
        for (; word != 0ull; word &= word - 1ull) {
            const int g = (w0 + lane) * 64 + (int)__builtin_ctzll(word);
            if (group_items) out[at] = (g << 4) | 15;
            else {
#pragma unroll
                for (int b = 0; b < 4; ++b) out[4 * at + b] = (g << 2) | b;
            }
            ++at;
        }
        base += __shfl(incl, 63, 64);
    }
    if (lane == 0) tcnt[tile] = group_items ? base : 4 * base;
}

__global__ __launch_bounds__(256) void exact_scout_rowneed_kernel(const float* __restrict__ X, long N, int D, int n_samples,
                                                                  const float* __restrict__ Cc, const float* __restrict__ rg,
                                                                  int n_groups, int* __restrict__ counts) {
    extern __shared__ float xs[];
    __shared__ float wmin[4];
    __shared__ int wcnt[4];
    const int tid = threadIdx.x, lane = tid & 63, wave = tid >> 6;
    const long step = N / n_samples;
    const float* x = X + ((long)blockIdx.x * step + step / 2) * D;
    for (int k = tid; k < D; k += 256) xs[k] = x[k];
    __syncthreads();
    auto dist = [&](int g) -> float {
        const float* c = Cc + (long)g * D;
        float q = 0.0f;
        if ((D & 3) == 0) {
            for (int k = 0; k < D; k += 4) {
                const f32x4 v = *(const f32x4*)(c + k);
#pragma unroll
                for (int j = 0; j < 4; ++j) { const float t = xs[k + j] - v[j]; q = __builtin_fmaf(t, t, q); }
            }
        } else {
            for (int k = 0; k < D; ++k) { const float t = xs[k] - c[k]; q = __builtin_fmaf(t, t, q); }
        }
        return __builtin_sqrtf(q);
    };
    float m = __builtin_inff();
    for (int g = tid; g < n_groups; g += 256) {
        const float r = rg[g];
        if (r >= 0.0f) m = __builtin_fminf(m, dist(g) + r);
    }
#pragma unroll
    for (int o = 32; o > 0; o >>= 1) m = __builtin_fminf(m, __shfl_xor(m, o, 64));
    if (lane == 0) wmin[wave] = m;
    __syncthreads();
    m = __builtin_fminf(__builtin_fminf(wmin[0], wmin[1]), __builtin_fminf(wmin[2], wmin[3]));
    int need = 0;
    for (int g = tid; g < n_groups; g += 256) {
        const float r = rg[g];
        if (r >= 0.0f) need += !(dist(g) - r > m) ? 1 : 0;
    }
#pragma unroll
    for (int o = 32; o > 0; o >>= 1) need += __shfl_xor(need, o, 64);
    if (lane == 0) wcnt[wave] = need;
    __syncthreads();
    if (tid == 0) { atomicAdd(counts, wcnt[0] + wcnt[1] + wcnt[2] + wcnt[3]); atomicAdd(counts + 1, 1); }
}

__global__ __launch_bounds__(256) void exact_sample_tiles_kernel(const int* __restrict__ order, const int* __restrict__ keys, long stride_tiles,
                                                                 int* __restrict__ order_out, int* __restrict__ keys_out) {
    const long src = (long)blockIdx.x * stride_tiles * SK_TILE + threadIdx.x;
    const long dst = (long)blockIdx.x * SK_TILE + threadIdx.x;
    static_assert(SK_TILE == 256, "one thread per row of a tile");
    order_out[dst] = order[src];
    keys_out[dst] = keys[src];
}

__global__ __launch_bounds__(256) void exact_scout_pos_kernel(unsigned long long* __restrict__ best64, long n, int K,
                                                              int* __restrict__ lastpos, const int* __restrict__ perm = nullptr) {
    const long p = (long)blockIdx.x * 256 + threadIdx.x;
    if (p >= n) return;
    const uint32_t u = (uint32_t)best64[p];
    const int pos = u < (uint32_t)K ? (int)u : 0;
    lastpos[p] = perm != nullptr ? perm[pos] : pos;
    best64[p] = ~0ull;
}

}
```

### xpysom_dask_amd/csrc/somhip.hip

```cpp
#include <hip/hip_runtime.h>

#include <cstring>

#include <dlfcn.h>

#include <cmath>
#include <cstdio>
#include <cstdlib>
#include <algorithm>
#include <atomic>
#include <cstring>
#include <string>
#include <utility>
#include <vector>

#include "../../include/somhip.h"
#include "../../include/somhip_test.h"
#include "bmu_bf16_k16.hpp"
#include "bmu_bf16_tiled.hpp"
#include "bmu_bf16_wide.hpp"
#include "bmu_exact.hpp"
#include "exact_skip.hpp"
#include "exact_policy.hpp"
#include "codebook_operands.hpp"
#include "exact_skip_wide.hpp"
#include "bmu_f32.hpp"
#include "bmu_f32_res.hpp"
#include "bmu_f32_tiled.hpp"
#include "bmu_pairwise.hpp"
#include "update.hpp"

using namespace somhip;

namespace {

thread_local std::string g_create_error;

const char* dev_env(const char* name) {
    static const bool on = [] { const char* v = std::getenv("SOM_TEST_HOOKS"); return v != nullptr && std::atoi(v) != 0; }();
    return on ? std::getenv(name) : nullptr;
}

struct EventPair { hipEvent_t a, b; int kernel; };

}

struct som_nccl_id { char internal[128]; };
struct RcclApi {
    void* lib = nullptr;
    int (*GetUniqueId)(som_nccl_id*) = nullptr;
    int (*CommInitRank)(void**, int, som_nccl_id, int) = nullptr;
    int (*AllReduce)(const void*, void*, size_t, int, int, void*, hipStream_t) = nullptr;
    int (*CommDestroy)(void*) = nullptr;
    const char* (*GetErrorString)(int) = nullptr;
};
static RcclApi g_rccl;
static std::string g_rccl_error;

static std::atomic<int64_t> g_dev_bytes{0};
template <typename T>
struct DevBuf {
    T* p = nullptr;
    size_t cap = 0;
    DevBuf() = default;
    DevBuf(const DevBuf&) = delete;
    DevBuf& operator=(const DevBuf&) = delete;
    DevBuf(DevBuf&& o) noexcept : p(o.p), cap(o.cap) { o.p = nullptr; o.cap = 0; }
    DevBuf& operator=(DevBuf&& o) noexcept {
        if (this != &o) { reset(); p = o.p; cap = o.cap; o.p = nullptr; o.cap = 0; }
        return *this;
    }
    ~DevBuf() { reset(); }
    void reset() {
        if (p) { (void)hipFree(p); g_dev_bytes -= (int64_t)(cap * sizeof(T)); }
        p = nullptr; cap = 0;
    }
    int alloc(som_handle* h, size_t n);
    int reserve(som_handle* h, size_t n, size_t round = 1) { return n <= cap ? 0 : alloc(h, (n + round - 1) / round * round); }
    operator T*() const { return p; }
};

struct som_handle {
    som_config cfg{};
    void* comm = nullptr;
    int comm_world = 1;
    hipStream_t comm_stream = nullptr;
    hipEvent_t ev_block = nullptr, ev_comm = nullptr;
    int X = 0, Y = 0, K = 0, D = 0, D1p = 0;
    int ks32 = 0;
    bool tiled = false;
    bool f16 = false;
    bool exact = false;
    bool ex_patch = false;
    bool ex_sub44 = false;
    DevBuf<int> ex_perm;
    DevBuf<int> ex_inv;
    DevBuf<float> Wp;
    DevBuf<float> wsq_p;
    struct ExactScratch {
        DevBuf<uint32_t> gmin;
        DevBuf<unsigned long long> gflags;
        long stride = 0;
        DevBuf<int> rowcnt;
        DevBuf<int> rowarg;
        DevBuf<float> seed;
        bool seed_on = true;
        bool seed_live = false;
        int two_round = -1;
        DevBuf<int> fb_list, fb_ids;
        DevBuf<int> ctr;
        DevBuf<int> plist;
        DevBuf<int4> tile_tab;
        long max_tiles = 0;
        DevBuf<float> fbX;
        PassCounters* pass_host = nullptr;
        hipEvent_t fb_ready = nullptr;
        int64_t rows_total = 0, rows_fallback = 0, chunks = 0;
        int64_t blocks_run = 0, blocks_total = 0;
        long pass_rows_override = 0;
        long hook_refuse_above = 0, hook_pairs = 0; bool hook_refuse_skip = false;
        long stride_cap = 0;
        long pairs = 64;
        int skip_mode = 1;
        policy::PlanState plan;
        policy::LaunchPlan lp;
        bool sub_blocks = true;
        struct SortedRows {
            long cap = 0;
            DevBuf<int> order;
            DevBuf<__bf16> Xb_s;
            DevBuf<__bf16> Xl_s;
            bool xl_filled = false;
            DevBuf<float> Xf_s, xsq_s, xerr_s, seed_s, sU_s;
            DevBuf<int> lastpos_s;
            bool lastpos_valid = false;
        } srt[2];
        int64_t lastpos_carried_epochs = 0;
        bool chain = true;
        bool cen_ready = false;
        long sk_stride = 0;
        int res_every = 0;
        DevBuf<int> sk_keys, sk_keys2, sk_vals;
        DevBuf<int> sk_tmp;
        bool refine_on = true;
        int grid_mult = 2;
        bool scout_on = true;
        DevBuf<int> scout_g;
        DevBuf<float> tq;
        double share_forecast = 1.0;
        struct Cost {
            hipEvent_t ev[8] = {};
            bool have = false;
        } cost;
        struct Centroids { DevBuf<float> Cc, rg, csq, cmax2; DevBuf<char> Cst;
                           DevBuf<char> Cst_plain;
                           int n_slots = 0, n_cstages = 0, n_img_stages = 0; } cen[2];
        DevBuf<unsigned long long> need, need2;
        DevBuf<int> glist, gcnt;
        DevBuf<int> tlist, tcnt;
        DevBuf<int2> tile_counts;
        DevBuf<int> tile_ticket;
        bool fuse_select = true;
        int64_t sel_fused_passes = 0, sel_launched_passes = 0, sel_ticket_tiles = 0;
        bool fuse_plan = true;
        int hook_plan_parts = 0;
        int64_t plan_fused_launches = 0, plan_split_launches = 0;
        DevBuf<int2> items;
        int item_slots = 0;
        int screen_slots = 0;
        bool item_queue = true;
        int item_len_pct = 125;
    } ex;
    int n_kchunks = 0;
    int n_ublocks = 0;
    bool tl_big = false;
    bool wide = false;
    int tl_bm = 128, tl_bn = 128, tl_xtile = 0, tl_wfrag = 0, tl_wtile = 0;
    int dp = 0;
    int stage_bytes = 0;
    int stage_units = 0;
    int nt = 1;
    bool swapped = false;
    int norm_p = 2;
    double norm_pr = 0.0;
    hipStream_t stream = nullptr;
    bool own_stream = false;

    DevBuf<float> W, wsq, SC, T, ACC, P1, P2;
    DevBuf<float> Ud;
    DevBuf<char> Wst;
    DevBuf<char> Wst_lo;
    DevBuf<char> Wfst;
    int fr_kg = 0, fr_stages = 0;
    DevBuf<char> Wfimg;
    DevBuf<char> ftX;
    int ft_kchunks = 0, ft_ublocks = 0;
    int n_stages = 0;
    operands::State ops;

    const float* Xd = nullptr;
    DevBuf<float> X_owned;
    long N = 0, Np = 0;
    DevBuf<int> bmu;
    bool bmu_valid = false;
    struct EarlyUpdate { bool armed = false, done = false; double sigma = 0, eta = 0; int neigh_f64 = 0; } early;
    DevBuf<unsigned long long> best64;
    int n_cus = 0;
    struct SegScratch {
        DevBuf<int> skey, srow;
        DevBuf<int> tmp;
        DevBuf<int> kA, kB;
        DevBuf<float> vA, vB;
        long cap = 0;
        DevBuf<int> cs_table;
        long cs_blocks = 0;
    };
    SegScratch seg;
    DevBuf<float> xsq;
    DevBuf<__bf16> Xb;
    DevBuf<float> xmax2;
    DevBuf<float> wn;
    DevBuf<float> wmax2;

    DevBuf<float> qX; DevBuf<int> qbmu, qbmu2; DevBuf<float> qxsq; DevBuf<__bf16> qXb;
    DevBuf<double> qX64;
    long qcap = 0;
    DevBuf<double> dsum;
    DevBuf<int> qe_list, qe_ids, qe_cnt; DevBuf<float> qe_X, qe_xsq;
    int64_t qe_rows = 0, qe_rows_sqrt = 0;
    struct Top2Scratch {
        bool on = true;
        DevBuf<float> m;
        DevBuf<int> excl;
        DevBuf<float> X, xsq;
        DevBuf<int> ids1, ids2;
        int64_t rows = 0, rows_f32 = 0;
    } t2;
    SegScratch st_seg;
    bool streaming = false;
    struct Slot {
        DevBuf<float> dX; DevBuf<__bf16> dXb; DevBuf<float> dxsq; DevBuf<int> dbmu;
        long cap = 0;
        hipEvent_t copied = nullptr, consumed = nullptr;
        bool used = false;
    } slot[2];
    hipStream_t copy_stream = nullptr;
    int slot_idx = 0;

    bool use_graph = false;
    bool capturing = false;
    hipGraphExec_t gexec = nullptr;
    unsigned long alloc_gen = 0, gexec_gen = 0;
    const void* gexec_rows = nullptr;
    long gexec_n = -1;
    int graph_warm = 0;
    DevBuf<NeighParams> np_dev;
    DevBuf<int2> bands;
    bool use_bands = true;

    int verify_rows = 0;
    bool verifying = false;
    DevBuf<int> vf_rows, vf_picks, vf_best, vf_bad;
    DevBuf<float> vf_X;
    int vf_cap = 0;
    int64_t verify_launches = 0, verify_rows_checked = 0;
    bool fuse_merge_prep = true;
    bool counting_sort = true;
    int env_bf16_parts = 0;
    int env_f32_parts = 0;
    bool debug = false;
    struct KernelSlots { const void* fn; size_t lds; int per_cu; };
    std::vector<KernelSlots> kernel_slots;
    int staged_blocks_done = -1;
    bool async_copies = false;
    int prof = 0;
    std::vector<EventPair> pending, pool;
    double ms[SOM_K_COUNT] = {0};
    int64_t launches[SOM_K_COUNT] = {0};

    std::string err;
};

namespace {

int fail(som_handle* h, const std::string& msg) {
    if (h) h->err = msg; else g_create_error = msg;
    return 1;
}
int fail_hip(som_handle* h, const char* what, hipError_t e) {
    return fail(h, std::string(what) + ": " + hipGetErrorString(e));
}

struct DeviceGuard {
    int prev = -1;
    bool moved = false;
    explicit DeviceGuard(const som_handle* h) {
        if (!h) return;
        if (hipGetDevice(&prev) != hipSuccess) prev = -1;
        if (prev != h->cfg.device) { (void)hipSetDevice(h->cfg.device); moved = true; }
    }
    ~DeviceGuard() { if (moved && prev >= 0) (void)hipSetDevice(prev); }
    DeviceGuard(const DeviceGuard&) = delete;
    DeviceGuard& operator=(const DeviceGuard&) = delete;
};

#define HIPCHK(h, call)                                              \
    do {                                                             \
        hipError_t e_ = (call);                                      \
        if (e_ != hipSuccess) return fail_hip((h), #call, e_);       \
    } while (0)

}

template <typename T>
int DevBuf<T>::alloc(som_handle* h, size_t n) {
    reset();
    if (n == 0) n = 1;
    if (h->capturing) return fail(h, "allocation during graph capture");
    if (hipError_t e = hipMalloc((void**)&p, n * sizeof(T)); e != hipSuccess) { p = nullptr; return fail_hip(h, "hipMalloc", e); }
// ... 860 lines not shown
}

const char* som_last_error(const som_handle* h) { return h ? h->err.c_str() : g_create_error.c_str(); }

int som_create(const som_config* cfg, som_handle** out) {
    if (!out) return fail(nullptr, "som_create: out is NULL");
    *out = nullptr;
    if (!cfg) return fail(nullptr, "som_create: cfg is NULL");
    if (cfg->x < 1 || cfg->y < 1 || cfg->input_len < 1) return fail(nullptr, "som_create: x, y, input_len must be >= 1");
    if ((long)cfg->x * cfg->y > (1L << 30)) return fail(nullptr, "som_create: map too large");
    if (cfg->distance < 0 || cfg->distance > SOM_DIST_NORM_P_NO_OPT) return fail(nullptr, "som_create: unknown distance id");
    if (cfg->norm_p < 0 || cfg->norm_p > PW_MAX_P) return fail(nullptr, "som_create: norm_p out of range (1..16)");
    if (cfg->norm_p_real != 0.0 && !(cfg->norm_p_real > 0.0 && cfg->norm_p_real <= 64.0))
        return fail(nullptr, "som_create: norm_p_real out of range (0 < p <= 64)");
    if (cfg->distance >= SOM_DIST_MANHATTAN && cfg->precision != SOM_PREC_F32 && cfg->precision != SOM_PREC_EXACT)
        return fail(nullptr, "som_create: manhattan / norm_p distances are float32 VALU kernels (precision f32)");
    if (cfg->neighborhood < 0 || cfg->neighborhood > SOM_NEIGH_TRIANGLE)
        return fail(nullptr, "som_create: unknown neighbourhood id");
    if (cfg->neighborhood == SOM_NEIGH_MEXICAN_HAT && cfg->compact_support && cfg->topology == SOM_TOPO_RECTANGULAR &&
        cfg->x != cfg->y)
        return fail(nullptr, "som_create: mexican_hat with compact_support needs a square map on the rectangular topology "
                             "(the reference's second mask on px does not broadcast otherwise, neighborhoods.py:70)");
    if (cfg->topology != SOM_TOPO_RECTANGULAR && cfg->topology != SOM_TOPO_HEXAGONAL)
        return fail(nullptr, "som_create: unknown topology id");
    if (cfg->topology == SOM_TOPO_HEXAGONAL && cfg->neighborhood == SOM_NEIGH_TRIANGLE)
        return fail(nullptr, "som_create: the hexagonal topology has no triangle neighbourhood (xpysom.py:271-279)");
    if (cfg->precision < SOM_PREC_F32 || cfg->precision > SOM_PREC_EXACT)
        return fail(nullptr, "som_create: unknown precision id");
    if (cfg->precision == SOM_PREC_RETIRED_2 || cfg->precision == SOM_PREC_RETIRED_4)
        return fail(nullptr, "som_create: the split-operand precisions (ids 2 and 4: 'bf16x3', 'f16x3') are retired -- "
                             "precision 'exact' returns float32's own BMUs, faster");
    if (cfg->precision != SOM_PREC_F32 && cfg->precision != SOM_PREC_EXACT) {
        if (cfg->distance == SOM_DIST_EUCLIDEAN_NO_OPT)
            return fail(nullptr, "som_create: bf16 precision implements 'euclidean' and 'cosine' "
                                 "('euclidean_no_opt' has the same argmin as 'euclidean')");
    }
    int ndev = 0;
    hipError_t e = hipGetDeviceCount(&ndev);
    if (e != hipSuccess || ndev < 1) return fail(nullptr, "som_create: no HIP device available");
    if (cfg->device < 0 || cfg->device >= ndev) return fail(nullptr, "som_create: device ordinal out of range");

    som_handle* h = new som_handle();
    h->cfg = *cfg;
    if (cfg->precision == SOM_PREC_EXACT) {
        if ((cfg->distance == SOM_DIST_EUCLIDEAN && cfg->input_len <= 128) ||
            ((cfg->distance == SOM_DIST_EUCLIDEAN || cfg->distance == SOM_DIST_COSINE) && cfg->input_len > 128)) h->exact = true;
        else h->cfg.precision = SOM_PREC_F32;
    }
    cfg = &h->cfg;
    h->X = cfg->x; h->Y = cfg->y; h->K = cfg->x * cfg->y; h->D = cfg->input_len;
    h->D1p = (int)round_up(h->D + 1, 4);
    h->norm_p = cfg->norm_p > 0 ? cfg->norm_p : 2;
    if (cfg->norm_p_real != 0.0 && (cfg->distance == SOM_DIST_NORM_P || cfg->distance == SOM_DIST_NORM_P_NO_OPT)) h->norm_pr = cfg->norm_p_real;
    h->ks32 = (int)cdiv(h->D, 32);
    h->f16 = cfg->precision == SOM_PREC_F16 || h->exact;
    h->tiled = (cfg->precision == SOM_PREC_BF16 || cfg->precision == SOM_PREC_F16 || h->exact) && h->D > 128;
    if (h->tiled) {
        h->tl_big = h->K >= 4096;
        if (h->tl_big) {
            using C = TileCfg<8, 2, 4>;
            h->tl_bm = C::BM; h->tl_bn = C::BN; h->tl_xtile = C::XTILE; h->tl_wfrag = C::WFRAG; h->tl_wtile = C::WTILE;
        } else {
            using C = TileCfg<4, 2, 2>;
            h->tl_bm = C::BM; h->tl_bn = C::BN; h->tl_xtile = C::XTILE; h->tl_wfrag = C::WFRAG; h->tl_wtile = C::WTILE;
        }
        h->n_kchunks = (int)cdiv((long)h->D, TL_BK);
        h->n_ublocks = (int)cdiv(h->K, h->tl_bn);
    }
    h->wide = h->tiled && h->tl_big && h->n_kchunks <= 25;
    if (const char* e = dev_env("SOM_BF16_WIDE")) if (std::atoi(e) == 0) h->wide = false;
    if (h->exact && h->tiled && !h->wide) {
        h->exact = false; h->f16 = false; h->tiled = false;
        h->cfg.precision = SOM_PREC_F32;
    }
    h->ex_patch = h->exact && h->K >= 2 * EX_GROUP;
    if (const char* e = dev_env("SOM_EXACT_PATCH")) if (std::atoi(e) == 0) h->ex_patch = false;
    h->ops = operands::State(operands::Config{h->cfg.precision != SOM_PREC_F32, h->exact, h->ex_patch, h->cfg.distance == SOM_DIST_COSINE,
                                              h->exact && !h->tiled, h->D <= 128});
    h->dp = h->tiled ? TL_BK * h->n_kchunks : 32 * h->ks32;
    h->stage_bytes = h->wide ? wd_stage_bytes(h->n_kchunks) : k16_stage_bytes(h->ks32);
    h->stage_units = h->wide ? WD_STAGE_UNITS : K16_STAGE_UNITS;
    h->nt = cfg->neighborhood == SOM_NEIGH_MEXICAN_HAT ? (cfg->compact_support ? 4 : 2) : 1;
    h->swapped = cfg->neighborhood == SOM_NEIGH_MEXICAN_HAT && cfg->compact_support && cfg->topology == SOM_TOPO_RECTANGULAR;
    if (cfg->topology == SOM_TOPO_HEXAGONAL && cfg->neighborhood != SOM_NEIGH_BUBBLE) h->nt *= cfg->compact_support ? 4 : 3;
    int rc = 0;
    auto bail = [&](int code) { g_create_error = h->err; som_destroy(h); return code; };
    DeviceGuard dev_guard(h);
    {
        int cur = -1;
        if (hipGetDevice(&cur) != hipSuccess || cur != cfg->device) return bail(fail(h, "hipSetDevice failed"));
    }
    {
        hipDeviceProp_t prop;
        if (hipGetDeviceProperties(&prop, cfg->device) == hipSuccess) h->n_cus = prop.multiProcessorCount;
    }
    if (cfg->stream) { h->stream = (hipStream_t)cfg->stream; }
    else {
        if (hipStreamCreateWithFlags(&h->stream, hipStreamNonBlocking) != hipSuccess)
            return bail(fail(h, "hipStreamCreate failed"));
        h->own_stream = true;
    }
    const size_t KD1 = (size_t)h->K * h->D1p;
    if ((rc = h->W.alloc(h, (size_t)h->K * h->D))) return bail(rc);
    if ((rc = h->wsq.alloc(h, (size_t)h->K))) return bail(rc);
    if (h->ex_patch) {
        if ((rc = h->Wp.alloc(h, (size_t)h->K * h->D))) return bail(rc);
        if ((rc = h->wsq_p.alloc(h, (size_t)h->K))) return bail(rc);
        if ((rc = h->ex_perm.alloc(h, (size_t)h->K))) return bail(rc);
        if ((rc = h->ex_inv.alloc(h, (size_t)h->K))) return bail(rc);
        std::vector<int> perm;
        bool blocks = true;
        if (const char* e = dev_env("SOM_EXACT_SUB44")) blocks = std::atoi(e) != 0;
        h->ex_sub44 = blocks && patch_order_blocks(h->X, h->Y);
        patch_order(h->X, h->Y, perm, blocks);
        std::vector<int> inv((size_t)h->K);
        for (int p = 0; p < h->K; ++p) inv[(size_t)perm[(size_t)p]] = p;
        if (hipMemcpy(h->ex_perm, perm.data(), (size_t)h->K * sizeof(int), hipMemcpyHostToDevice) != hipSuccess ||
            hipMemcpy(h->ex_inv, inv.data(), (size_t)h->K * sizeof(int), hipMemcpyHostToDevice) != hipSuccess)
            return bail(fail(h, "hipMemcpy of the patch-order tables failed"));
    }
    if ((rc = h->SC.alloc(h, KD1 + (size_t)h->K))) return bail(rc);
    if ((rc = h->Ud.alloc(h, (size_t)h->nt * h->K))) return bail(rc);
    if ((rc = h->T.alloc(h, KD1 * h->nt))) return bail(rc);
    if ((rc = h->ACC.alloc(h, KD1))) return bail(rc);
    if ((rc = h->P1.alloc(h, (size_t)h->nt * h->Y * h->Y))) return bail(rc);
    if ((rc = h->P2.alloc(h, (size_t)h->X * h->nt * h->X))) return bail(rc);
    if ((rc = h->dsum.alloc(h, 1))) return bail(rc);
    {
        if ((rc = h->np_dev.alloc(h, 1))) return bail(rc);
        if (const char* e = std::getenv("SOM_GRAPH")) h->use_graph = std::atoi(e) != 0;
        if (const char* e = dev_env("SOM_BF16_PARTS")) h->env_bf16_parts = std::atoi(e);
        if (const char* e = dev_env("SOM_F32_PARTS")) h->env_f32_parts = std::atoi(e);
        h->debug = std::getenv("SOM_DEBUG") != nullptr;
        if (const char* e = std::getenv("SOM_VERIFY")) h->verify_rows = std::max(0, std::atoi(e));
        if (const char* e = dev_env("SOM_EXACT_PASS_ROWS")) h->ex.pass_rows_override = std::atol(e);
        if (const char* e = dev_env("SOM_EXACT_DEBUG_REFUSE_ABOVE")) h->ex.hook_refuse_above = std::atol(e);
        if (const char* e = dev_env("SOM_EXACT_PAIRS")) h->ex.hook_pairs = std::max(1L, std::atol(e));
        h->ex.hook_refuse_skip = dev_env("SOM_EXACT_DEBUG_REFUSE_SKIP") != nullptr;
        if (const char* e = dev_env("SOM_EXACT_TWO_ROUND")) h->ex.two_round = std::atoi(e) != 0 ? 1 : 0;
        if (const char* e = dev_env("SOM_EXACT_SEED")) h->ex.seed_on = std::atoi(e) != 0;
        if (const char* e = std::getenv("SOM_EXACT_SKIP")) h->ex.skip_mode = std::atoi(e);
        if (const char* e = std::getenv("SOM_EXACT_TOP2")) h->t2.on = std::atoi(e) != 0;
        if (const char* e = dev_env("SOM_EXACT_SUBBLOCKS")) h->ex.sub_blocks = std::atoi(e) != 0;
        if (const char* e = dev_env("SOM_EXACT_REFINE")) h->ex.refine_on = std::atoi(e) != 0;
        if (const char* e = dev_env("SOM_EXACT_QUEUE")) { h->ex.item_queue = std::atoi(e) != 0; if (std::atoi(e) >= 25) h->ex.item_len_pct = std::atoi(e); }
        if (const char* e = dev_env("SOM_EXACT_SCOUT")) h->ex.scout_on = std::atoi(e) != 0;
        if (const char* e = dev_env("SOM_EXACT_GRID_MULT")) h->ex.grid_mult = std::max(1, std::atoi(e));
        if (const char* e = dev_env("SOM_EXACT_RESORT")) h->ex.res_every = std::max(0, std::atoi(e));
        if (const char* e = dev_env("SOM_ASYNC_COPIES")) h->async_copies = std::atoi(e) != 0;
        if (const char* e = dev_env("SOM_FUSE_MERGE")) h->fuse_merge_prep = std::atoi(e) != 0;
        if (const char* e = dev_env("SOM_EXACT_CHAIN")) h->ex.chain = std::atoi(e) != 0;
        if (const char* e = dev_env("SOM_EXACT_FUSE_SELECT")) h->ex.fuse_select = std::atoi(e) != 0;
        if (const char* e = dev_env("SOM_EXACT_FUSE_PLAN")) h->ex.fuse_plan = std::atoi(e) != 0;
        if (const char* e = dev_env("SOM_EXACT_PLAN_PARTS")) h->ex.hook_plan_parts = std::max(0, std::atoi(e));
        if (const char* e = dev_env("SOM_COUNTING_SORT")) h->counting_sort = std::atoi(e) != 0;
        h->use_bands = h->X > 256 || h->Y > 256;
        if (const char* e = dev_env("SOM_NO_BANDS")) h->use_bands = std::atoi(e) == 0;
        const size_t nb = (size_t)h->nt * (cdiv(h->Y, LM_BM) + cdiv(h->X, LM_BM));
        if ((rc = h->bands.alloc(h, nb))) return bail(rc);
    }
    if (hipMemsetAsync(h->W, 0, (size_t)h->K * h->D * sizeof(float), h->stream) != hipSuccess ||
        hipMemsetAsync(h->T, 0, KD1 * h->nt * sizeof(float), h->stream) != hipSuccess ||
        hipMemsetAsync(h->ACC, 0, KD1 * sizeof(float), h->stream) != hipSuccess)
        return bail(fail(h, "hipMemsetAsync failed"));
    if (h->D > 128) {
        h->ft_kchunks = (int)cdiv(h->D, FT_BK);
        h->ft_ublocks = (int)cdiv(h->K, FT_BN);
        if ((rc = h->Wfimg.alloc(h, (size_t)h->ft_ublocks * h->ft_kchunks * FT_WTILE))) return bail(rc);
    }
    if (h->D <= 128) {
        int kg = 1;
        while (kg * 8 < h->D) kg *= 2;
        h->fr_kg = kg;
        h->fr_stages = (int)cdiv(h->K, FR_STAGE_UNITS);
        if ((rc = h->Wfst.alloc(h, (size_t)h->fr_stages * fr_stage_bytes(kg)))) return bail(rc);
    }
    if (h->cfg.precision != SOM_PREC_F32) {
        h->n_stages = (int)cdiv(h->K, h->stage_units);
        size_t bytes = (size_t)h->n_stages * h->stage_bytes;
        if (h->tiled && !h->wide) bytes = (size_t)h->n_ublocks * h->n_kchunks * h->tl_wtile;
        if ((rc = h->Wst.alloc(h, bytes))) return bail(rc);
        if (h->exact && !h->tiled) {
            if ((rc = h->Wst_lo.alloc(h, bytes))) return bail(rc);
            if (hipMemsetAsync(h->Wst_lo, 0, bytes, h->stream) != hipSuccess) return bail(fail(h, "hipMemsetAsync failed"));
        }
        if ((rc = h->xmax2.alloc(h, 2))) return bail(rc);
        if ((rc = h->wn.alloc(h, (size_t)h->K))) return bail(rc);
        if ((rc = h->wmax2.alloc(h, 2))) return bail(rc);
        if (hipMemsetAsync(h->Wst, 0, bytes, h->stream) != hipSuccess) return bail(fail(h, "hipMemsetAsync failed"));
    }
    if (hipStreamSynchronize(h->stream) != hipSuccess) return bail(fail(h, "hipStreamSynchronize failed"));
    *out = h;
    return 0;
}

void som_destroy(som_handle* h) {
    if (!h) return;
    DeviceGuard dev_guard(h);
    (void)som_comm_destroy(h);
    if (h->comm_stream) (void)hipStreamDestroy(h->comm_stream);
    if (h->ev_block) (void)hipEventDestroy(h->ev_block);
    if (h->ev_comm) (void)hipEventDestroy(h->ev_comm);
    if (h->stream) (void)hipStreamSynchronize(h->stream);
    if (h->gexec) (void)hipGraphExecDestroy(h->gexec);
    for (auto& ep : h->pending) { (void)hipEventDestroy(ep.a); (void)hipEventDestroy(ep.b); }
    for (auto& ep : h->pool) { (void)hipEventDestroy(ep.a); (void)hipEventDestroy(ep.b); }
    if (h->ex.cost.have) for (auto& e : h->ex.cost.ev) (void)hipEventDestroy(e);
    if (h->ex.fb_ready) (void)hipEventDestroy(h->ex.fb_ready);
    for (auto& sl : h->slot) {
        if (sl.copied) (void)hipEventDestroy(sl.copied);
        if (sl.consumed) (void)hipEventDestroy(sl.consumed);
    }
    if (h->ex.pass_host) (void)hipHostFree(h->ex.pass_host);
    if (h->copy_stream) (void)hipStreamDestroy(h->copy_stream);
    if (h->own_stream && h->stream) (void)hipStreamDestroy(h->stream);
    delete h;
}

int som_set_weights(som_handle* h, const float* w_host) {
    DeviceGuard dev_guard(h);
    if (!h || !w_host) return fail(h, "som_set_weights: NULL argument");
    if (h->f16 && !h->exact && h->cfg.distance != SOM_DIST_COSINE) {
        for (long k = 0; k < h->K; ++k) {
            double q = 0.0;
            for (int d = 0; d < h->D; ++d) { const double v = w_host[k * h->D + d]; q += v * v; }
            if (q > (double)HALF_MAX * HALF_MAX && q <= 1.0e300)
                return fail(h, "som_set_weights: precision 'f16' needs units of norm <= 65504 (float16 range): scale the data, or use 'bf16' / 'f32'");
        }
    }
    if (int rc = h2d_blocking(h, h->W, w_host, (size_t)h->K * h->D * sizeof(float))) return rc;
    HIPCHK(h, hipStreamSynchronize(h->stream));
    h->ops.codebook_replaced();
    return 0;
}

int som_get_weights(som_handle* h, float* w_host) {
    DeviceGuard dev_guard(h);
    if (!h || !w_host) return fail(h, "som_get_weights: NULL argument");
    return d2h_blocking(h, w_host, h->W, (size_t)h->K * h->D * sizeof(float));
}

static int adopt_rows(som_handle* h, int64_t n_rows) {
    h->bmu.reset(); h->xsq.reset(); h->Xb.reset();
    h->bmu_valid = false;
    h->ex.plan.order_lost();
    h->ex.srt[0].lastpos_valid = false;
    h->seg = som_handle::SegScratch{};
    h->N = n_rows;
    h->Np = round_up(n_rows, ROW_PAD);
    if (n_rows > 0x7fffffffL) return fail(h, "som_set_data: more than 2^31-1 rows per GPU");
    if (int rc = h->bmu.alloc(h, (size_t)n_rows)) return rc;
    if (n_rows > 0)
        if (int rc = seg_reserve(h, h->seg, n_rows)) return rc;
    const bool bf_cos_tiled = h->cfg.precision != SOM_PREC_F32 && h->cfg.distance == SOM_DIST_COSINE && h->tiled;
    if (needs_xsq(h) || bf_cos_tiled) {
        if (int rc = h->xsq.alloc(h, (size_t)n_rows * (h->exact ? 2 : 1))) return rc;
        if (needs_xsq(h)) if (int rc = row_sq(h, h->Xd, n_rows, h->xsq)) return rc;
    }
    if (h->cfg.precision != SOM_PREC_F32 && n_rows > 0) {
        if (int rc = h->Xb.alloc(h, (size_t)h->Np * h->dp)) return rc;
        if (int rc = prep_rows_bf16(h, h->Xd, n_rows, h->Np, h->Xb, h->xmax2, h->xsq)) return rc;
    }
    HIPCHK(h, hipStreamSynchronize(h->stream));
    if (h->f16 && !h->exact && n_rows > 0) {
        float m2 = 0.0f;
        if (int rc = d2h_blocking(h, &m2, h->xmax2, sizeof(float))) return rc;
        if (!(m2 <= HALF_MAX * HALF_MAX))
            return fail(h, "som_set_data: precision 'f16' needs rows of norm <= 65504 (float16 range): scale the data, or use 'bf16' / 'f32'");
    }
    if (h->exact && n_rows > 0) {
        bool ok = exact_reserve(h, n_rows) == 0;
        if (ok && exact_skip_wanted(h) && !h->wide)
            ok = exact_skip_reserve(h, h->ex.srt[0], n_rows, h->ex.stride) == 0;
        if (!ok) { (void)hipGetLastError(); h->err.clear(); }
    }
    return 0;
}

int som_set_data(som_handle* h, const float* x_host, int64_t n_rows) {
    DeviceGuard dev_guard(h);
    if (!h || n_rows < 0 || (!x_host && n_rows > 0)) return fail(h, "som_set_data: bad argument");
    h->Xd = nullptr;
    if (int rc = h->X_owned.alloc(h, (size_t)n_rows * h->D)) return rc;
    if (n_rows > 0)
        if (int rc = h2d_blocking(h, h->X_owned, x_host, (size_t)n_rows * h->D * sizeof(float))) return rc;
    h->Xd = h->X_owned;
    return adopt_rows(h, n_rows);
}

int som_set_data_device(som_handle* h, const void* x_dev, int64_t n_rows) {
    DeviceGuard dev_guard(h);
    if (!h || n_rows < 0 || (!x_dev && n_rows > 0)) return fail(h, "som_set_data_device: bad argument");
    h->X_owned.reset();
    h->Xd = (const float*)x_dev;
    return adopt_rows(h, n_rows);
}

int som_sync_producer(som_handle* h, uint64_t stream, int32_t has_stream) {
    DeviceGuard dev_guard(h);
    if (!h) return 1;
    if (!has_stream) { HIPCHK(h, hipDeviceSynchronize()); return 0; }
    hipStream_t st = stream == 1 ? (hipStream_t)0 : stream == 2 ? hipStreamPerThread : (hipStream_t)(uintptr_t)stream;
    HIPCHK(h, hipStreamSynchronize(st));
    return 0;
}

// ... 663 lines not shown
    case 6:
        if (h->ex.cen_ready)
            for (int lv = 0; lv < (h->wide ? 1 : 2) && rc == 0; ++lv) {
                auto& c = h->ex.cen[lv];
                if ((rc = add(c.Cc, (size_t)c.n_slots * h->D * sizeof(float)))) break;
                if ((rc = add(c.rg, (size_t)c.n_slots * sizeof(float)))) break;
                if ((rc = add(c.csq, (size_t)c.n_slots * sizeof(float)))) break;
                rc = add(c.cmax2, 2 * sizeof(float));
            }
        break;
    case 7: rc = add(h->ex_patch ? (const float*)h->Wp : (const float*)h->W, (size_t)h->K * h->D * sizeof(float)); break;
    default: return fail(h, "som_debug_operand_crc: unknown buffer");
    }
    if (rc) return rc;
    *out = hash;
    return 0;
}

int som_debug_exact_centroids(som_handle* h, int32_t level, float* C_out, float* r_out, float* csq_out, int32_t* n_slots_out) {
    DeviceGuard dev_guard(h);
    if (!h || !n_slots_out) return fail(h, "som_debug_exact_centroids: NULL argument");
    if (!h->ex.cen_ready) return fail(h, "som_debug_exact_centroids: the handle holds no centroids (no launch has planned yet)");
    if (level < 0 || level >= (h->wide ? 1 : 2)) return fail(h, "som_debug_exact_centroids: no such level");
    const auto& c = h->ex.cen[level];
    *n_slots_out = c.n_slots;
    HIPCHK(h, hipStreamSynchronize(h->stream));
    if (C_out) if (int rc = d2h_blocking(h, C_out, c.Cc, (size_t)c.n_slots * h->D * sizeof(float))) return rc;
    if (r_out) if (int rc = d2h_blocking(h, r_out, c.rg, (size_t)c.n_slots * sizeof(float))) return rc;
    if (csq_out) if (int rc = d2h_blocking(h, csq_out, c.csq, (size_t)c.n_slots * sizeof(float))) return rc;
    return 0;
}

int som_policy_eval(int32_t which, const double* costs, const double* args, int32_t* out) {
    if (!costs || !args || !out) return 1;
    policy::Costs c;
    c.full_total = costs[0]; c.full_screen = costs[1]; c.plan_total = costs[2]; c.plan_over = costs[3]; c.plan_over_scout = costs[4];
    c.blk_ms = costs[5]; c.l2_ms_group = costs[6]; c.l2_ratio = costs[7]; c.sort_ms = costs[8];
    switch (which) {
    case 0: *out = policy::commit_scouted_plan(c, args[0], args[1]); return 0;
    case 1: *out = policy::level2_from_sample(c, args[0], args[1], args[2]); return 0;
    case 2: *out = policy::level2_pays(c, args[0], args[1]); return 0;
    case 3: *out = policy::sort_paid(c, args[0], args[1], args[2], (int)args[3]); return 0;
    case 4: *out = policy::plan_idle(c, args[0]); return 0;
    case 5: *out = policy::scout_continues(c, args[0], args[1], args[2]); return 0;
    case 6: *out = policy::rows_worth_a_scout(args[0], args[1], args[2]); return 0;
    }
    return 1;
}

int som_policy_replay(int32_t n_launches, const double* script, double* out) {
    if (n_launches < 0 || !script || !out) return 1;
    policy::PlanState st;
    for (int32_t i = 0; i < n_launches; ++i) {
        const double* in = script + (size_t)i * SOM_POLICY_REPLAY_IN;
        double* o = out + (size_t)i * SOM_POLICY_REPLAY_OUT;
        policy::LaunchFacts f;
        f.resident = in[0] != 0.0; f.have_last = in[1] != 0.0; f.rows = (const void*)(uintptr_t)in[2]; f.n_rows = (long)in[3];
        f.can_skip = in[4] != 0.0; f.scout_ok = in[5] != 0.0; f.wide = in[6] != 0.0; f.wide_can = in[7] != 0.0; f.wide_scout_ok = in[8] != 0.0;
        f.l2_fits_lds = in[9] != 0.0; f.have_lo_image = in[10] != 0.0; f.blocks_per_row = in[11];
        f.skip_mode = (int)in[12]; f.refine_on = in[13] != 0.0; f.sub_blocks = in[14] != 0.0; f.res_every = (int)in[15];
        policy::LaunchPlan p = st.begin(f);
        const bool asked_rows = p.estimate;
        const bool row_no = asked_rows && st.rows_sampled(in[16], p);
        const bool asked_tiles = p.estimate && p.sample_tiles && in[17] >= 0.0;
        const bool tile_no = asked_tiles && st.tiles_sampled(in[17], in[18], f, p);
        policy::LaunchOutcome oc;
        oc.t_total = in[19]; oc.t_screen = in[20]; oc.t_l2 = in[21]; oc.t_sort = in[22];
        oc.screen_timed = p.time_phases; oc.l2_timed = p.time_phases && p.skip && p.level2; oc.sort_timed = p.time_phases && p.skip && p.resort;
        oc.blocks_total = (int64_t)in[24];
        oc.blocks_run = p.skip ? (int64_t)in[23] : oc.blocks_total;
        oc.groups_run = p.skip ? (int64_t)in[25] : oc.blocks_total / policy::TILES_PER_GROUP;
        oc.pairs_in = (int64_t)in[26]; oc.pairs_out = p.refine ? (int64_t)in[27] : 0; oc.scout_wins = (p.skip && p.scout && f.have_last) ? (int64_t)in[28] : 0;
        st.end(f, p, oc);
        o[0] = p.skip; o[1] = p.resort; o[2] = p.scout; o[3] = p.level2; o[4] = p.estimate; o[5] = p.sample_tiles; o[6] = p.refine; o[7] = p.time_phases;
        o[8] = asked_rows; o[9] = asked_tiles; o[10] = row_no; o[11] = tile_no;
        for (int k = 0; k < 2; ++k) {
            const policy::Pause& ps = st.pause(k == 0);
            o[12 + 3 * k] = ps.cooldown; o[13 + 3 * k] = ps.idle; o[14 + 3 * k] = ps.pause;
        }
    }
    return 0;
}

int som_operands_replay(const int32_t* config, int32_t n_events, const int32_t* script, int32_t* out) {
    if (!config || n_events < 0 || !script || !out) return 1;
    const operands::Config cfg{config[0] != 0, config[1] != 0, config[2] != 0, config[3] != 0, config[4] != 0, config[5] != 0};
    if (!cfg.valid()) return 1;
    operands::State st(cfg);
    for (int32_t i = 0; i < n_events; ++i) {
        const int32_t* in = script + (size_t)i * SOM_OPERANDS_REPLAY_IN;
        int32_t* o = out + (size_t)i * SOM_OPERANDS_REPLAY_OUT;
        if (in[1] < 0 || in[1] > 2) return 1;
        const operands::Request rq = in[1] == 0 ? operands::Request::Search : in[1] == 1 ? operands::Request::F32Units : operands::Request::ExactScreen;
        operands::Rebuilds r;
        switch (in[0]) {
        case 0: st.codebook_replaced(); break;
        case 1: st.merged_plain(); break;
        case 2: if (!cfg.half || cfg.exact) return 1; st.merged_half_fused(); break;
        case 3: if (!cfg.resident) return 1; st.merged_exact_fused(in[2] != 0); break;
        case 4: if (in[2] != 0 && !cfg.resident) return 1; r = st.decide(rq, in[2] != 0); st.commit(r); break;
        case 5: r.flush = st.take_pending_image(&r.flush_cm); break;
        case 6: if (cfg.exact) return 1; st.graph_replayed(rq); break;
        case 7: r = st.decide_wsq(); st.commit(r); break;
        default: return 1;
        }
        o[0] = r.wsq; o[1] = r.permute; o[2] = r.f32; o[3] = r.f32_patch; o[4] = r.half; o[5] = r.skip_norms; o[6] = r.deferred; o[7] = r.cm;
        o[8] = r.flush; o[9] = r.flush_cm;
        o[10] = st.f32_in_patch_order(); o[11] = st.image_pending(); o[12] = st.centroids_fresh(); o[13] = st.patch_copy_in_step();
    }
    return 0;
}

int som_debug_mfma16(som_handle* h, const uint16_t* a_host, const uint16_t* b_host, const float* c_host, float* d_host,
                     int32_t is_f16) {
    DeviceGuard dev_guard(h);
    if (!h || !a_host || !b_host || !c_host || !d_host) return fail(h, "som_debug_mfma16: NULL argument");
    DevBuf<uint16_t> a, b;
    DevBuf<float> c, d;
    int rc = 0;
    if ((rc = a.alloc(h, 512)) || (rc = b.alloc(h, 512)) || (rc = c.alloc(h, 256)) || (rc = d.alloc(h, 256))) return rc;
    if (h2d_blocking(h, a, a_host, 1024) || h2d_blocking(h, b, b_host, 1024) || h2d_blocking(h, c, c_host, 1024)) return 1;
    if (is_f16) debug_mfma16_kernel<F16><<<dim3(1), dim3(64), 0, h->stream>>>(a, b, c, d);
    else debug_mfma16_kernel<Bf16><<<dim3(1), dim3(64), 0, h->stream>>>(a, b, c, d);
    return d2h_blocking(h, d_host, d, 1024);
}

int som_debug_device_bytes(int64_t* out) {
    if (!out) return 1;
    *out = g_dev_bytes.load();
    return 0;
}

int som_debug_exact_chain_stats(som_handle* h, int64_t* carried_epochs) {
    if (!h || !carried_epochs) return fail(h, "som_debug_exact_chain_stats: NULL argument");
    *carried_epochs = h->ex.lastpos_carried_epochs;
    return 0;
}

int som_debug_exact_select_stats(som_handle* h, int64_t* fused_passes, int64_t* launched_passes, int64_t* ticket_tiles) {
    if (!h || !fused_passes || !launched_passes || !ticket_tiles) return fail(h, "som_debug_exact_select_stats: NULL argument");
    *fused_passes = h->ex.sel_fused_passes;
    *launched_passes = h->ex.sel_launched_passes;
    *ticket_tiles = h->ex.sel_ticket_tiles;
    return 0;
}

int som_debug_exact_plan_stats(som_handle* h, int64_t* fused_launches, int64_t* split_launches) {
    if (!h || !fused_launches || !split_launches) return fail(h, "som_debug_exact_plan_stats: NULL argument");
    *fused_launches = h->ex.plan_fused_launches;
    *split_launches = h->ex.plan_split_launches;
    return 0;
}

int som_debug_exact_last_plan(som_handle* h, int32_t* out8) {
    if (!h || !out8) return fail(h, "som_debug_exact_last_plan: NULL argument");
    const policy::LaunchPlan& p = h->ex.lp;
    out8[0] = p.skip; out8[1] = p.resort; out8[2] = p.scout; out8[3] = p.level2; out8[4] = p.estimate; out8[5] = p.sample_tiles;
    out8[6] = p.refine; out8[7] = p.time_phases;
    return 0;
}

int som_debug_qe_stats(som_handle* h, int64_t* rows, int64_t* rows_sqrt) {
    if (!h || !rows || !rows_sqrt) return fail(h, "som_debug_qe_stats: NULL argument");
    *rows = h->qe_rows;
    *rows_sqrt = h->qe_rows_sqrt;
    return 0;
}

int som_debug_stamps(som_handle* h, int64_t n_pairs, uint64_t* out_host) {
    DeviceGuard dev_guard(h);
    if (!h) return 1;
#ifdef SOM_STAMPS
    static unsigned long long* buf = nullptr;
    static int64_t cap = 0;
    HIPCHK(h, hipStreamSynchronize(h->stream));
    if (out_host) {
        if (n_pairs > cap) return fail(h, "som_debug_stamps: more pairs than the buffer holds");
        HIPCHK(h, hipMemcpy(out_host, buf, (size_t)n_pairs * 16, hipMemcpyDeviceToHost));
        return 0;
    }
    if (buf) { (void)hipFree(buf); buf = nullptr; cap = 0; }
    if (n_pairs > 0) {
        HIPCHK(h, hipMalloc((void**)&buf, (size_t)n_pairs * 16));
        HIPCHK(h, hipMemset(buf, 0, (size_t)n_pairs * 16));
        cap = n_pairs;
    }
    HIPCHK(h, hipMemcpyToSymbol(HIP_SYMBOL(g_som_stamps), &buf, sizeof(buf)));
    return 0;
#else
    (void)n_pairs; (void)out_host;
    return fail(h, "som_debug_stamps: this library was built without -DSOM_STAMPS (tools/stamps.py builds the diagnostic one)");
#endif
}

int som_patch_order(int32_t x, int32_t y, int32_t* perm_out) {
    if (x <= 0 || y <= 0 || !perm_out || (int64_t)x * y > 0x7fffffffLL) return 1;
    std::vector<int> perm;
    patch_order(x, y, perm);
    std::copy(perm.begin(), perm.end(), perm_out);
    return 0;
}

int som_exact_stats(som_handle* h, int64_t* rows, int64_t* rows_fallback, int64_t* passes) {
    if (!h) return 1;
    if (rows) *rows = h->ex.rows_total;
    if (rows_fallback) *rows_fallback = h->ex.rows_fallback;
    if (passes) *passes = h->ex.chunks;
    return 0;
}

int som_exact_top2_stats(som_handle* h, int64_t* rows, int64_t* rows_f32) {
    if (!h || !rows || !rows_f32) return fail(h, "som_exact_top2_stats: NULL argument");
    *rows = h->t2.rows; *rows_f32 = h->t2.rows_f32;
    return 0;
}

int som_exact_skip_stats(som_handle* h, int64_t* blocks_run, int64_t* blocks_total) {
    if (!h || !blocks_run || !blocks_total) return 1;
    *blocks_run = h->ex.blocks_run; *blocks_total = h->ex.blocks_total;
    return 0;
}

int som_exact_resident_stats(som_handle* h, int64_t* planned_epochs, int64_t* sorts) {
    if (!h || !planned_epochs || !sorts) return 1;
    *planned_epochs = h->ex.plan.stats().planned; *sorts = h->ex.plan.stats().resorts;
    return 0;
}

int som_exact_scout_stats(som_handle* h, int64_t* scouted_launches, int64_t* transient_planned) {
    if (!h || !scouted_launches || !transient_planned) return 1;
    *scouted_launches = h->ex.plan.stats().scouted; *transient_planned = h->ex.plan.stats().tr_planned;
    return 0;
}

int som_exact_refine_stats(som_handle* h, int64_t* pairs_in, int64_t* pairs_out) {
    if (!h || !pairs_in || !pairs_out) return 1;
    *pairs_in = h->ex.plan.stats().pairs_refined_in; *pairs_out = h->ex.plan.stats().pairs_refined_out;
    return 0;
}

int som_exact_last_counts(som_handle* h, int32_t* counts_out, int64_t n) {
    DeviceGuard dev_guard(h);
    if (!h || !counts_out || n < 0) return fail(h, "som_exact_last_counts: bad argument");
    if (!h->exact || n > h->ex.stride) return fail(h, "som_exact_last_counts: no screen pass of that many rows");
    if (int rc = d2h_blocking(h, counts_out, h->ex.rowcnt, (size_t)n * sizeof(int32_t))) return rc;
    return 0;
}

int som_sync(som_handle* h) {
    DeviceGuard dev_guard(h);
    if (!h) return 1;
    HIPCHK(h, hipStreamSynchronize(h->stream));
    return 0;
}

int som_profile_enable(som_handle* h, int32_t on) {
    DeviceGuard dev_guard(h);
    if (!h) return 1;
    if (!on) if (int rc = resolve_profile(h)) return rc;
    h->prof = on == 2 ? 2 : on != 0;
    return 0;
}

int som_profile_get(som_handle* h, int32_t kernel, double* total_ms, int64_t* launches) {
    DeviceGuard dev_guard(h);
    if (!h || kernel < 0 || kernel >= SOM_K_COUNT) return fail(h, "som_profile_get: bad argument");
    if (int rc = resolve_profile(h)) return rc;
    if (total_ms) *total_ms = h->ms[kernel];
    if (launches) *launches = h->launches[kernel];
    return 0;
}

int som_profile_reset(som_handle* h) {
    DeviceGuard dev_guard(h);
    if (!h) return 1;
    if (int rc = resolve_profile(h)) return rc;
    for (int i = 0; i < SOM_K_COUNT; ++i) { h->ms[i] = 0; h->launches[i] = 0; }
    return 0;
}

}
```

### xpysom_dask_amd/engine.py

```python
import ctypes as C

import numpy as np

from . import _lib


class SomHipError(RuntimeError):
    pass


def _f32(a):
    return np.ascontiguousarray(a, dtype=np.float32)


class HipEngine:
    def __init__(self, x, y, input_len, *, distance="euclidean", neighborhood="gaussian",
                 std_coeff=0.5, compact_support=False, precision="exact", device=0, stream=None,
                 topology="rectangular", norm_p=0, norm_p_real=0.0):
        self._lib = _lib.load()
        self._h = None
        self.K, self.D = int(x) * int(y), int(input_len)
        self.x, self.y = int(x), int(y)
        self.n_rows = 0
        self._keepalive = None
# ... 138 lines not shown
        self._check(self._lib.som_stream_begin(self._h))
        for chunk in chunks:
            chunk = _f32(chunk)
            if chunk.ndim != 2 or chunk.shape[1] != self.D:
                raise ValueError("chunk must be (n, %d), got %r" % (self.D, chunk.shape))
            self._check(self._lib.som_stream_rows(self._h, self._fp(chunk), chunk.shape[0]))
        self._check(self._lib.som_stream_end(self._h, float(sigma), float(eta), int(bool(neigh_f64))))
        self.sync()

    def epoch_fetch(self, want_bmu=True):
        num = np.empty((self.K, self.D), dtype=np.float32)
        den = np.empty((self.K,), dtype=np.float32)
        bmu = np.empty((self.n_rows,), dtype=np.int32) if want_bmu else None
        self._check(self._lib.som_epoch_fetch(self._h, self._fp(num), self._fp(den),
                                              self._ip(bmu) if want_bmu else None))
        return num, den, bmu

    def accum_device_ptr(self):
        p, n = C.c_void_p(), C.c_int64()
        self._check(self._lib.som_accum_device_ptr(self._h, C.byref(p), C.byref(n)))
        return p.value, n.value

    def stream_ptr(self):
        p = C.c_void_p()
        self._check(self._lib.som_get_stream(self._h, C.byref(p)))
        return int(p.value or 0)

    def accum_tensor(self):
        import torch
        ptr, n = self.accum_device_ptr()

        class _Alias:
            __cuda_array_interface__ = {"shape": (n,), "typestr": "<f4", "data": (ptr, False),
                                        "version": 2, "strides": None}
        return torch.as_tensor(_Alias(), device=torch.device("cuda", self.device))

    def bmu(self, x, quantization=False):
        x = _f32(x)
        if x.ndim != 2 or x.shape[1] != self.D:
            raise ValueError("x must be (n, %d), got %r" % (self.D, x.shape))
        ids = np.empty((x.shape[0],), dtype=np.int32)
        mode = _lib.SOM_BMU_QUANTIZATION if quantization else _lib.SOM_BMU_ACTIVATION
        self._check(self._lib.som_bmu(self._h, self._fp(x), x.shape[0], mode, self._ip(ids)))
        return ids

    def bmu_device(self, dev_ptr, n_rows, quantization=False):
        ids = np.empty((int(n_rows),), dtype=np.int32)
        mode = _lib.SOM_BMU_QUANTIZATION if quantization else _lib.SOM_BMU_ACTIVATION
        self._check(self._lib.som_bmu_device(self._h, C.c_void_p(dev_ptr), int(n_rows), mode, self._ip(ids)))
        return ids

    def quantization_error_device(self, dev_ptr, n_rows):
        out = C.c_double()
        self._check(self._lib.som_quantization_error_device(self._h, C.c_void_p(dev_ptr), int(n_rows), C.byref(out)))
        return out.value

    def bmu_f64(self, x):
        x = np.ascontiguousarray(x, dtype=np.float64)
        if x.ndim != 2 or x.shape[1] != self.D:
            raise ValueError("x must be (n, %d), got %r" % (self.D, x.shape))
        ids = np.empty((x.shape[0],), dtype=np.int32)
        self._check(self._lib.som_bmu_f64(self._h, x.ctypes.data_as(C.POINTER(C.c_double)), x.shape[0], self._ip(ids)))
        return ids

    def bmu_top2(self, x):
        x = _f32(x)
        if x.ndim != 2 or x.shape[1] != self.D:
            raise ValueError("x must be (n, %d), got %r" % (self.D, x.shape))
        a = np.empty((x.shape[0],), dtype=np.int32)
        b = np.empty((x.shape[0],), dtype=np.int32)
        self._check(self._lib.som_bmu_top2(self._h, self._fp(x), x.shape[0], self._ip(a), self._ip(b)))
        return a, b

    def bmu_top2_device(self, dev_ptr, n_rows):
        a = np.empty((int(n_rows),), dtype=np.int32)
        b = np.empty((int(n_rows),), dtype=np.int32)
        self._check(self._lib.som_bmu_top2_device(self._h, C.c_void_p(dev_ptr), int(n_rows), self._ip(a), self._ip(b)))
        return a, b

    def distance_matrix(self, x, quantization=False):
        x = _f32(x)
        if x.ndim != 2 or x.shape[1] != self.D:
            raise ValueError("x must be (n, %d), got %r" % (self.D, x.shape))
        out = np.empty((x.shape[0], self.K), dtype=np.float32)
        mode = _lib.SOM_BMU_QUANTIZATION if quantization else _lib.SOM_BMU_ACTIVATION
        self._check(self._lib.som_distance_matrix(self._h, self._fp(x), x.shape[0], mode, self._fp(out)))
        return out

    def quantization_error(self, x):
        x = _f32(x)
        out = C.c_double()
        self._check(self._lib.som_quantization_error(self._h, self._fp(x), x.shape[0], C.byref(out)))
        return out.value

    def set_verify(self, n_rows):
        self._check(self._lib.som_set_verify(self._h, int(n_rows)))

    def verify_stats(self):
        a, b = C.c_int64(), C.c_int64()
        self._check(self._lib.som_verify_stats(self._h, C.byref(a), C.byref(b)))
        return a.value, b.value

    def debug_corrupt_operands(self, which=3):
        self._check(self._lib.som_debug_corrupt_operands(self._h, int(which)))

    def debug_exact_centroids(self, level):
        n = C.c_int32()
        self._check(self._lib.som_debug_exact_centroids(self._h, int(level), None, None, None, C.byref(n)))
        cen = np.empty((n.value, self.D), dtype=np.float32)
        rad = np.empty((n.value,), dtype=np.float32)
        csq = np.empty((n.value,), dtype=np.float32)
        self._check(self._lib.som_debug_exact_centroids(self._h, int(level), self._fp(cen), self._fp(rad), self._fp(csq), C.byref(n)))
        return cen, rad, csq

    def debug_mfma16(self, a, b, c, f16=True):
        a = np.ascontiguousarray(a).view(np.uint16).reshape(16, 32)
        b = np.ascontiguousarray(b).view(np.uint16).reshape(32, 16)
        c = np.ascontiguousarray(c, dtype=np.float32).reshape(16, 16)
        d = np.empty((16, 16), dtype=np.float32)
        self._check(self._lib.som_debug_mfma16(self._h, a.ctypes.data_as(C.c_void_p), b.ctypes.data_as(C.c_void_p),
                                               self._fp(c), self._fp(d), int(bool(f16))))
        return d

    def exact_stats(self):
        a, b, c = C.c_int64(), C.c_int64(), C.c_int64()
        self._check(self._lib.som_exact_stats(self._h, C.byref(a), C.byref(b), C.byref(c)))
        return a.value, b.value, c.value

    def qe_stats(self):
        a, b = C.c_int64(), C.c_int64()
        self._check(self._lib.som_debug_qe_stats(self._h, C.byref(a), C.byref(b)))
        return a.value, b.value

    def exact_top2_stats(self):
        a, b = C.c_int64(), C.c_int64()
        self._check(self._lib.som_exact_top2_stats(self._h, C.byref(a), C.byref(b)))
        return a.value, b.value

    def exact_chain_stats(self):
        a = C.c_int64()
        self._check(self._lib.som_debug_exact_chain_stats(self._h, C.byref(a)))
        return a.value

    def exact_select_stats(self):
        a, b, c = C.c_int64(), C.c_int64(), C.c_int64()
        self._check(self._lib.som_debug_exact_select_stats(self._h, C.byref(a), C.byref(b), C.byref(c)))
        return a.value, b.value, c.value

    def exact_plan_stats(self):
        a, b = C.c_int64(), C.c_int64()
        self._check(self._lib.som_debug_exact_plan_stats(self._h, C.byref(a), C.byref(b)))
        return a.value, b.value

    def exact_last_plan(self):
        out = (C.c_int32 * 8)()
        self._check(self._lib.som_debug_exact_last_plan(self._h, out))
        return dict(zip(("skip", "resort", "scout", "level2", "estimate", "sample_tiles", "refine", "time_phases"), (bool(v) for v in out)))

    def exact_skip_stats(self):
        a, b = C.c_int64(), C.c_int64()
        self._check(self._lib.som_exact_skip_stats(self._h, C.byref(a), C.byref(b)))
        return a.value, b.value

    def exact_resident_stats(self):
        a, b = C.c_int64(), C.c_int64()
        self._check(self._lib.som_exact_resident_stats(self._h, C.byref(a), C.byref(b)))
        return a.value, b.value

    def exact_scout_stats(self):
        a, b = C.c_int64(), C.c_int64()
        self._check(self._lib.som_exact_scout_stats(self._h, C.byref(a), C.byref(b)))
        return a.value, b.value

    def exact_refine_stats(self):
        a, b = C.c_int64(), C.c_int64()
        self._check(self._lib.som_exact_refine_stats(self._h, C.byref(a), C.byref(b)))
        return a.value, b.value

    def exact_last_counts(self, n):
        out = np.empty((int(n),), dtype=np.int32)
        self._check(self._lib.som_exact_last_counts(self._h, self._ip(out), int(n)))
        return out

    def sync(self):
        self._check(self._lib.som_sync(self._h))

    def profile_enable(self, on=True):
        self._check(self._lib.som_profile_enable(self._h, 2 if on == "bmu" else int(bool(on))))

    def profile_reset(self):
        self._check(self._lib.som_profile_reset(self._h))

    def profile_get(self, kernel):
        ms, n = C.c_double(), C.c_int64()
        self._check(self._lib.som_profile_get(self._h, _lib.SOM_KERNELS[kernel], C.byref(ms), C.byref(n)))
        return ms.value, n.value
```

Measured before the change: 545.7 million.

## Fold plan threshold into MFMA accumulator so pruning test becomes a sign check

Splits each row's pruning threshold P into three low-precision parts, scaled by a power of two, and feeds them as extra MFMA operand columns multiplied by -c. The accumulator then already holds the value minus the threshold, and the per-row test is reduced to an unsigned max plus a sign-bit compare, replacing the per-subblock float compares. The bound is widened slightly to cover the extra rounding. The change also lets the fused plan kernel run for the KS32=4 bf16 case by widening the per-entry LDS slot. Folding is on by default and can be turned off for f16 via an env var, at the cost of extra MFMA k-slots and threshold splitting work.

```diff
diff --git a/xpysom_dask_amd/_lib.py b/xpysom_dask_amd/_lib.py
--- a/xpysom_dask_amd/_lib.py
+++ b/xpysom_dask_amd/_lib.py
@@ -79,6 +79,8 @@
     "som_debug_exact_chain_stats": (C.c_int, [_H, C.POINTER(C.c_int64)]),
     "som_debug_exact_select_stats": (C.c_int, [_H, C.POINTER(C.c_int64), C.POINTER(C.c_int64), C.POINTER(C.c_int64)]),
     "som_debug_exact_plan_stats": (C.c_int, [_H, C.POINTER(C.c_int64), C.POINTER(C.c_int64)]),
+    "som_debug_exact_plan_fold_stats": (C.c_int, [_H, C.POINTER(C.c_int64), C.POINTER(C.c_int64)]),
+    "som_debug_plan_split": (C.c_int, [C.c_int32, C.c_int64, C.POINTER(C.c_float), C.POINTER(C.c_float), C.POINTER(C.c_float)]),
     "som_debug_exact_last_plan": (C.c_int, [_H, C.POINTER(C.c_int32)]),
     "som_policy_eval": (C.c_int, [C.c_int32, C.POINTER(C.c_double), C.POINTER(C.c_double), C.POINTER(C.c_int32)]),
     "som_policy_replay": (C.c_int, [C.c_int32, C.POINTER(C.c_double), C.POINTER(C.c_double)]),
diff --git a/xpysom_dask_amd/csrc/exact_host.hpp b/xpysom_dask_amd/csrc/exact_host.hpp
--- a/xpysom_dask_amd/csrc/exact_host.hpp
+++ b/xpysom_dask_amd/csrc/exact_host.hpp
@@ -420,7 +420,8 @@
                                                                   n_items, n_items + 1, ex.item_len_pct);
 }
 
-template <int KS32, class E> constexpr bool plan_fused_fits() { return !(KS32 == 4 && std::is_same<E, Bf16>::value); }
+template <int KS32, class E> constexpr bool plan_fused_fits() { return true; }
+template <class E> bool plan_folds(bool asked) { return asked || !std::is_same<E, F16>::value; }
 template <class E>
 int exact_skip_plan(som_handle* h, som_handle::ExactScratch::SortedRows& sr, long s0, long n, const float* xmax2, const ExactBound& eb,
                     const int* lastpos2, bool time_l2 = false) {
@@ -439,8 +440,9 @@
     const bool l2 = ex.lp.level2;
     const int force = ex.skip_mode == 3 ? 1 : 0;
     const __bf16* Xs = sr.Xb_s + s0 * h->dp;
-    const size_t lds = lds2 + (size_t)c0.n_cstages * 8 + (size_t)SK_TILE * sizeof(float);
+    const size_t lds = lds2 + (size_t)c0.n_cstages * 8 + (size_t)SK_TILE * 8;
     const bool fits = h->ks32 != 4 || plan_fused_fits<4, E>();
+    const bool fold = plan_folds<E>(ex.plan_fold);
     if (ex.fuse_plan && ex.chain && l2 && lastpos2 == nullptr && pgrid.y == 1 && !time_l2 && lds <= 160 * 1024 && fits) {
         PlanListsOut lo;
         lo.n_groups = (int)cdiv(h->K, EX_GROUP);
@@ -450,41 +452,48 @@
         lo.slots = ex.item_queue ? (ex.screen_slots > 0 ? ex.screen_slots : ex.item_slots) : 0;
         lo.items = ex.item_queue ? ex.items + 8 : nullptr;
         lo.n_items = (int*)ex.items.p; lo.item_ctr = lo.n_items + 1; lo.len_pct = ex.item_len_pct;
+#define SOM_PLAN_FUSED_RUN(k, F) { \
+        { int pc; if (int rc = kernel_per_cu(h, (const void*)exact_plan_fused_kernel<k, E, F>, 64 * K16_NW, lds, &pc)) return rc; } \
+        exact_plan_fused_kernel<k, E, F><<<dim3((unsigned)tiles), block, lds, h->stream>>>(Xs, n, c0.Cst, c0.n_cstages, c0.cmax2, c1.Cst, c1.n_slots, \
+            c1.cmax2, sr.xsq_s + s0, sr.xerr_s + s0, xmax2, h->wmax2, h->wmax2 + 1, eb, sr.lastpos_s + s0, h->Wst, sr.seed_s + s0, force, lo); }
 #define SOM_PLAN_FUSED_CASE(k) case k: if constexpr (plan_fused_fits<k, E>()) { \
-        { int pc; if (int rc = kernel_per_cu(h, (const void*)exact_plan_fused_kernel<k, E>, 64 * K16_NW, lds, &pc)) return rc; } \
-        exact_plan_fused_kernel<k, E><<<dim3((unsigned)tiles), block, lds, h->stream>>>(Xs, n, c0.Cst, c0.n_cstages, c0.cmax2, c1.Cst, c1.n_slots, \
-            c1.cmax2, sr.xsq_s + s0, sr.xerr_s + s0, xmax2, h->wmax2, h->wmax2 + 1, eb, sr.lastpos_s + s0, h->Wst, sr.seed_s + s0, force, lo); \
+        if (fold) SOM_PLAN_FUSED_RUN(k, true) else if constexpr (std::is_same<E, F16>::value) SOM_PLAN_FUSED_RUN(k, false) \
         } break;
         switch (h->ks32) {
         SOM_PLAN_FUSED_CASE(1) SOM_PLAN_FUSED_CASE(2) SOM_PLAN_FUSED_CASE(3) SOM_PLAN_FUSED_CASE(4)
         default: return fail(h, "exact: block skipping supports input_len <= 128");
         }
 #undef SOM_PLAN_FUSED_CASE
+#undef SOM_PLAN_FUSED_RUN
         ++ex.plan_fused_launches;
+        ++(fold ? ex.plan_folded : ex.plan_compared);
         HIPCHK(h, hipGetLastError());
         return 0;
     }
     ++ex.plan_split_launches;
+    ++(fold ? ex.plan_folded : ex.plan_compared);
     unsigned long long* const need2_clear = l2 && ex.chain ? ex.need2.p : nullptr;
     if (l2 && !ex.chain) HIPCHK(h, hipMemsetAsync(ex.need2, 0, (size_t)tiles * c1.n_cstages * sizeof(unsigned long long), h->stream));
-#define SOM_PLAN_CASE(k) case k: { \
-        { int pc; if (int rc = kernel_per_cu(h, (const void*)exact_plan_kernel<k, E, false>, 64 * K16_NW, lds1, &pc)) return rc; } \
-        exact_plan_kernel<k, E, false><<<pgrid, block, lds1, h->stream>>>(Xs, n, c0.Cst, c0.n_cstages, c0.rg, c0.n_slots, \
+#define SOM_PLAN_RUN(k, F) { \
+        { int pc; if (int rc = kernel_per_cu(h, (const void*)exact_plan_kernel<k, E, false, F>, 64 * K16_NW, lds1, &pc)) return rc; } \
+        exact_plan_kernel<k, E, false, F><<<pgrid, block, lds1, h->stream>>>(Xs, n, c0.Cst, c0.n_cstages, c0.rg, c0.n_slots, \
             sr.xsq_s + s0, sr.xerr_s + s0, sr.sU_s + s0, xmax2, c0.cmax2, h->wmax2, h->wmax2 + 1, eb, ex.need, sr.lastpos_s + s0, \
             h->Wst, sr.seed_s + s0, nullptr, 0, force, lastpos2, lastpos2 != nullptr ? &ctr->scout_wins : nullptr, need2_clear); \
         if (l2) { \
             if (time_l2) (void)hipEventRecord(ex.cost.ev[3], h->stream); \
-            { int pc; if (int rc = kernel_per_cu(h, (const void*)exact_plan_kernel<k, E, true>, 64 * K16_NW, lds2, &pc)) return rc; } \
-            exact_plan_kernel<k, E, true><<<dim3((unsigned)tiles, pgrid.y), block, lds2, h->stream>>>(Xs, n, c1.Cst, c1.n_cstages, c1.rg, c1.n_slots, \
+            { int pc; if (int rc = kernel_per_cu(h, (const void*)exact_plan_kernel<k, E, true, F>, 64 * K16_NW, lds2, &pc)) return rc; } \
+            exact_plan_kernel<k, E, true, F><<<dim3((unsigned)tiles, pgrid.y), block, lds2, h->stream>>>(Xs, n, c1.Cst, c1.n_cstages, c1.rg, c1.n_slots, \
                 sr.xsq_s + s0, sr.xerr_s + s0, sr.sU_s + s0, xmax2, c1.cmax2, h->wmax2, h->wmax2 + 1, eb, ex.need2, nullptr, \
                 nullptr, nullptr, ex.need, c0.n_cstages, force); \
             if (time_l2) (void)hipEventRecord(ex.cost.ev[4], h->stream); \
-        } } break;
+        } }
+#define SOM_PLAN_CASE(k) case k: if (fold) SOM_PLAN_RUN(k, true) else if constexpr (std::is_same<E, F16>::value) SOM_PLAN_RUN(k, false) break;
     switch (h->ks32) {
     SOM_PLAN_CASE(1) SOM_PLAN_CASE(2) SOM_PLAN_CASE(3) SOM_PLAN_CASE(4)
     default: return fail(h, "exact: block skipping supports input_len <= 128");
     }
 #undef SOM_PLAN_CASE
+#undef SOM_PLAN_RUN
     exact_plan_lists(h, tiles, c0.n_cstages, l2 ? ex.need2.p : nullptr);
     HIPCHK(h, hipGetLastError());
     return 0;
diff --git a/xpysom_dask_amd/csrc/exact_skip.hpp b/xpysom_dask_amd/csrc/exact_skip.hpp
--- a/xpysom_dask_amd/csrc/exact_skip.hpp
+++ b/xpysom_dask_amd/csrc/exact_skip.hpp
@@ -243,6 +243,68 @@
     return f;
 }
 
+struct PlanParts { float p1, p2, p3; };
+template <class EL> struct PlanPartFmt;
+template <> struct PlanPartFmt<F16> {
+    static constexpr int M = 10, CMIN = -14, CMAX = 15;
+    static constexpr float MINN = 0x1p-14f, MAXV = 65504.0f;
+};
+template <> struct PlanPartFmt<Bf16> {
+    static constexpr int M = 7, CMIN = -100, CMAX = 100;
+    static constexpr float MINN = 0x1p-126f, MAXV = 0x1.FEp127f;
+};
+__host__ __device__ inline float plan_part_round(float v, int M, bool up) {
+    uint32_t b = __builtin_bit_cast(uint32_t, v);
+    const int sh = 23 - M;
+    const uint32_t low = (1u << sh) - 1u;
+    if (up) { if ((b >> 31) == 0u) b += low; }
+    else b += (low >> 1) + ((b >> sh) & 1u);
+    b &= ~low;
+    return __builtin_bit_cast(float, b);
+}
+template <class EL>
+__host__ __device__ inline float plan_fold_scale(float s_bmag) {
+    using F = PlanPartFmt<EL>;
+    const float m = s_bmag * (1.01f / 65504.0f);
+    if (!(m > 0.0f) || !(m < 3.0e38f)) return 1.0f;
+    const uint32_t b = __builtin_bit_cast(uint32_t, m);
+    int e = (int)(b >> 23) - 127 + ((b & 0x7FFFFFu) != 0u ? 1 : 0);
+    e = e > F::CMAX ? F::CMAX : e < F::CMIN ? F::CMIN : e;
+    return __builtin_bit_cast(float, (uint32_t)(e + 127) << 23);
+}
+template <class EL>
+__host__ __device__ inline PlanParts plan_split_threshold(float P, float c) {
+    using F = PlanPartFmt<EL>;
+    const float inf = __builtin_inff();
+    if (!(P == P) || P == inf) return PlanParts{inf, 0.0f, 0.0f};
+    if (P == -inf) return PlanParts{-inf, 0.0f, 0.0f};
+    {
+        uint32_t b = __builtin_bit_cast(uint32_t, P);
+        if ((b << 1) == 0u) b = 1u; else b = (b >> 31) == 0u ? b + 1u : b - 1u;
+        P = __builtin_bit_cast(float, b);
+        if (P == inf) return PlanParts{inf, 0.0f, 0.0f};
+    }
+    const float rc = __builtin_bit_cast(float, (uint32_t)(254 - (int)(__builtin_bit_cast(uint32_t, c) >> 23)) << 23);
+    const float t = P * rc;
+    if (P > 0.0f && !(t >= F::MINN)) return PlanParts{0.0f, 0.0f, F::MINN};
+    if (P <= 0.0f && !(t <= -F::MINN)) return PlanParts{0.0f, 0.0f, 0.0f};
+    if (!(t < 3.0e38f)) return PlanParts{inf, 0.0f, 0.0f};
+    PlanParts o;
+    o.p1 = plan_part_round(t, F::M, false);
+    if (o.p1 > F::MAXV) return PlanParts{inf, 0.0f, 0.0f};
+    if (o.p1 < -F::MAXV) return PlanParts{-F::MAXV, 0.0f, 0.0f};
+    const float r1 = t - o.p1;
+    o.p2 = plan_part_round(r1, F::M, false);
+    if (__builtin_fabsf(o.p2) < F::MINN) o.p2 = 0.0f;
+    const float r2 = r1 - o.p2;
+    if (r2 > 0.0f) o.p3 = r2 < F::MINN ? F::MINN : plan_part_round(r2, F::M, true);
+    else {
+        o.p3 = plan_part_round(r2, F::M, true);
+        if (__builtin_fabsf(o.p3) < F::MINN) o.p3 = 0.0f;
+    }
+    return o;
+}
+
 __device__ __forceinline__ uint32_t row16_or(uint32_t v) {
     v |= (uint32_t)__builtin_amdgcn_update_dpp(0, (int)v, 0x121, 0xF, 0xF, false);
     v |= (uint32_t)__builtin_amdgcn_update_dpp(0, (int)v, 0x122, 0xF, 0xF, false);
@@ -381,7 +443,7 @@
     return su;
 }
 
-template <int KS32>
+template <int KS32, bool FOLD>
 __device__ __forceinline__ void plan_row_threshold(const ExactBound& eb, const ExactScales& sc, bool in_pass, float q, float xe, float su,
                                                    float& P, float& bx) {
     const float S = sc.sx * sc.sw;
@@ -395,31 +457,46 @@
         }
     }
     bx = up_to_half(sc.sx * sU * (1.0f + 1.0f / 1024.0f));
-    P = A + 0.5f * S * (1.0f + 1.0f / 1024.0f) * sU * sU * (1.0f + 0x1p-20f) + (float)(24 * (KS32 + 1)) * 0x1p-23f * S * sc.bmag;
+    P = A + 0.5f * S * (1.0f + 1.0f / 1024.0f) * sU * sU * (1.0f + 0x1p-20f) + (float)(24 * (KS32 + 1) + (FOLD ? 28 : 0)) * 0x1p-23f * S * sc.bmag;
     if (!(bx < 3.0e38f) || !(P == P)) P = __builtin_inff();
     if (A == -__builtin_inff()) P = -__builtin_inff();
 }
-template <class EL>
-__device__ __forceinline__ typename V8<typename EL::T>::t plan_extra_step(float bx) {
+template <class EL, bool FOLD>
+__device__ __forceinline__ typename V8<typename EL::T>::t plan_extra_step(float bx, float P, float c) {
     using E = typename EL::T;
     typename V8<E>::t v;
 #pragma unroll
     for (int jj = 0; jj < 8; ++jj) v[jj] = (E)0.0f;
-    if (((threadIdx.x & 63) >> 4) == 0 && bx < 3.0e38f) v[0] = (E)bx;
+    if (((threadIdx.x & 63) >> 4) == 0) {
+        if (bx < 3.0e38f) v[0] = (E)bx;
+        if constexpr (FOLD) {
+            const PlanParts pp = plan_split_threshold<EL>(P, c);
+            v[1] = (E)pp.p1; v[2] = (E)pp.p2; v[3] = (E)pp.p3;
+        }
+    }
     return v;
 }
-
-template <int KS32, class EL>
+template <class EL>
+struct PlanTest {
+    float P[K16_SB];
+    typename EL::T negc;
+};
+
+template <int KS32, class EL, bool FOLD>
 __device__ __forceinline__ void plan_run_tile(int j, const typename V8<typename EL::T>::t (&a)[KS32], const f32x4& wv, float rneg,
                                               const typename V8<typename EL::T>::t (&xf)[K16_SB][KS32],
-                                              const typename V8<typename EL::T>::t (&xe)[K16_SB], const float (&P)[K16_SB],
+                                              const typename V8<typename EL::T>::t (&xe)[K16_SB], const PlanTest<EL>& pt,
                                               uint32_t& lane_bits) {
     using E = typename EL::T;
     using bf16x8 = typename V8<E>::t;
+    const float (&P)[K16_SB] = pt.P;
     bf16x8 ae;
 #pragma unroll
     for (int jj = 0; jj < 8; ++jj) ae[jj] = (E)0.0f;
-    if (((threadIdx.x & 63) >> 4) == 0) ae[0] = (E)rneg;
+    if (((threadIdx.x & 63) >> 4) == 0) {
+        ae[0] = (E)rneg;
+        if constexpr (FOLD) { ae[1] = pt.negc; ae[2] = pt.negc; ae[3] = pt.negc; }
+    }
     f32x4 acc[K16_SB];
 #pragma unroll
     for (int sb = 0; sb < K16_SB; ++sb) acc[sb] = wv;
@@ -431,10 +508,17 @@
     for (int sb = 0; sb < K16_SB; ++sb) acc[sb] = mfma16(ae, xe[sb], acc[sb]);
 #pragma unroll
     for (int r = 0; r < 4; ++r) {
-        bool nd = false;
-#pragma unroll
-        for (int sb = 0; sb < K16_SB; ++sb) nd = nd || !(acc[sb][r] > P[sb]);
-        lane_bits |= nd ? (1u << (4 * j + r)) : 0u;
+        if constexpr (FOLD) {
+            uint32_t m = __float_as_uint(acc[0][r]);
+#pragma unroll
+            for (int sb = 1; sb < K16_SB; ++sb) { const uint32_t u = __float_as_uint(acc[sb][r]); m = u > m ? u : m; }
+            lane_bits |= m > 0x7F800000u ? (1u << (4 * j + r)) : 0u;
+        } else {
+            bool nd = false;
+#pragma unroll
+            for (int sb = 0; sb < K16_SB; ++sb) nd = nd || !(acc[sb][r] > P[sb]);
+            lane_bits |= nd ? (1u << (4 * j + r)) : 0u;
+        }
     }
 }
 template <int KS32, class EL>
@@ -448,10 +532,10 @@
     rneg = wq[64 + t * 16 + (lane & 15)];
 }
 
-template <int KS32, class EL>
+template <int KS32, class EL, bool FOLD>
 __device__ __forceinline__ void plan_walk_level1(const char* __restrict__ Cst, int s_begin, int s_end, char* smem, unsigned long long* nl,
                                                  const typename V8<typename EL::T>::t (&xf)[K16_SB][KS32],
-                                                 const typename V8<typename EL::T>::t (&xe)[K16_SB], const float (&P)[K16_SB]) {
+                                                 const typename V8<typename EL::T>::t (&xe)[K16_SB], const PlanTest<EL>& P) {
     using bf16x8 = typename V8<typename EL::T>::t;
     constexpr int STAGE = k16_stage_bytes(KS32);
     constexpr int PIECES = K16_T * KS32 + 1;
@@ -474,12 +558,12 @@
         float rnA, rnB;
         plan_load_tile<KS32, EL>(st, 0, aA, wvA, rnA);
         plan_load_tile<KS32, EL>(st, 1, aB, wvB, rnB);
-        plan_run_tile<KS32, EL>(0, aA, wvA, rnA, xf, xe, P, lane_bits);
+        plan_run_tile<KS32, EL, FOLD>(0, aA, wvA, rnA, xf, xe, P, lane_bits);
         plan_load_tile<KS32, EL>(st, 2, aA, wvA, rnA);
-        plan_run_tile<KS32, EL>(1, aB, wvB, rnB, xf, xe, P, lane_bits);
+        plan_run_tile<KS32, EL, FOLD>(1, aB, wvB, rnB, xf, xe, P, lane_bits);
         plan_load_tile<KS32, EL>(st, 3, aB, wvB, rnB);
-        plan_run_tile<KS32, EL>(2, aA, wvA, rnA, xf, xe, P, lane_bits);
-        plan_run_tile<KS32, EL>(3, aB, wvB, rnB, xf, xe, P, lane_bits);
+        plan_run_tile<KS32, EL, FOLD>(2, aA, wvA, rnA, xf, xe, P, lane_bits);
+        plan_run_tile<KS32, EL, FOLD>(3, aB, wvB, rnB, xf, xe, P, lane_bits);
         const uint32_t any_row = row16_or(lane_bits);
         if (col == 0 && any_row != 0u) {
             const uint32_t lo = ((any_row & 15u) | (((any_row >> 4) & 15u) << 16)) << (4 * quad);
@@ -503,10 +587,10 @@
     if (lane == 0) *act_n = cnt;
 }
 
-template <int KS32, class EL>
+template <int KS32, class EL, bool FOLD>
 __device__ __forceinline__ void plan_walk_level2(const char* __restrict__ Cst, const int* act, int b0, int e0, char* smem,
                                                  unsigned long long* nl, const typename V8<typename EL::T>::t (&xf)[K16_SB][KS32],
-                                                 const typename V8<typename EL::T>::t (&xe)[K16_SB], const float (&P)[K16_SB]) {
+                                                 const typename V8<typename EL::T>::t (&xe)[K16_SB], const PlanTest<EL>& P) {
     using bf16x8 = typename V8<typename EL::T>::t;
     constexpr int STAGE = k16_stage_bytes(KS32);
     static_assert(K16_NW == 4, "a wave per tile fills the slot's tail");
@@ -552,14 +636,14 @@
         const bool h1 = c0 + 4 < e0, h2 = c0 + 8 < e0, h3 = c0 + 12 < e0;
         plan_load_tile<KS32, EL>(st, 0, aA, wvA, rnA);
         if (h1) plan_load_tile<KS32, EL>(st, 1, aB, wvB, rnB);
-        plan_run_tile<KS32, EL>(0, aA, wvA, rnA, xf, xe, P, lane_bits);
+        plan_run_tile<KS32, EL, FOLD>(0, aA, wvA, rnA, xf, xe, P, lane_bits);
         if (h1) {
             if (h2) plan_load_tile<KS32, EL>(st, 2, aA, wvA, rnA);
-            plan_run_tile<KS32, EL>(1, aB, wvB, rnB, xf, xe, P, lane_bits);
+            plan_run_tile<KS32, EL, FOLD>(1, aB, wvB, rnB, xf, xe, P, lane_bits);
             if (h2) {
                 if (h3) plan_load_tile<KS32, EL>(st, 3, aB, wvB, rnB);
-                plan_run_tile<KS32, EL>(2, aA, wvA, rnA, xf, xe, P, lane_bits);
-                if (h3) plan_run_tile<KS32, EL>(3, aB, wvB, rnB, xf, xe, P, lane_bits);
+                plan_run_tile<KS32, EL, FOLD>(2, aA, wvA, rnA, xf, xe, P, lane_bits);
+                if (h3) plan_run_tile<KS32, EL, FOLD>(3, aB, wvB, rnB, xf, xe, P, lane_bits);
             }
         }
         const uint32_t any_row = row16_or(lane_bits);
@@ -578,7 +662,7 @@
     }
 }
 
-template <int KS32, class EL, bool LEVEL2>
+template <int KS32, class EL, bool LEVEL2, bool FOLD>
 __global__ __launch_bounds__(64 * K16_NW, LEVEL2 ? 3 : 2) void exact_plan_kernel(const __bf16* __restrict__ Xb, long N,
                                                                     const char* __restrict__ Cst, int n_cstages,
                                                                     const float* __restrict__ rg, int n_slots,
@@ -606,9 +690,11 @@
 
     bf16x8 xf[K16_SB][KS32];
     bf16x8 xe[K16_SB];
-    float P[K16_SB];
+    PlanTest<EL> pt;
     const ExactScales sc = ex_scales(xmax2, cmax2, cmax2 + 1);
     const ExactScales sw = ex_scales(xmax2, wmax2, werr2);
+    const float cf = plan_fold_scale<EL>(sc.sx * sc.sw * sc.bmag);
+    pt.negc = (typename EL::T)(-cf);
 #pragma unroll
     for (int sb = 0; sb < K16_SB; ++sb) {
         const long row = wave_s0 + sb * 16 + col;
@@ -625,8 +711,8 @@
             }
         }
         float bx;
-        plan_row_threshold<KS32>(eb, sc, row < N, q, xer, su, P[sb], bx);
-        xe[sb] = plan_extra_step<EL>(bx);
+        plan_row_threshold<KS32, FOLD>(eb, sc, row < N, q, xer, su, pt.P[sb], bx);
+        xe[sb] = plan_extra_step<EL, FOLD>(bx, pt.P[sb], cf);
     }
 
     int* act = (int*)(smem + 2 * STAGE);
@@ -639,7 +725,7 @@
         const int c_all = (n_act + 15) / 16;
         const int b0 = 16 * (int)((long)c_all * blockIdx.y / gridDim.y);
         const int e0 = min(n_act, 16 * (int)((long)c_all * (blockIdx.y + 1) / gridDim.y));
-        plan_walk_level2<KS32, EL>(Cst, act, b0, e0, smem, nl, xf, xe, P);
+        plan_walk_level2<KS32, EL, FOLD>(Cst, act, b0, e0, smem, nl, xf, xe, pt);
         __syncthreads();
         for (int i = tid; i < n_cstages; i += 64 * K16_NW)
             if (nl[i] != 0ull) atomicOr(need + (long)blockIdx.x * n_cstages + i, nl[i]);
@@ -647,7 +733,7 @@
     }
     const int s_begin = (int)((long)n_cstages * blockIdx.y / gridDim.y);
     const int s_end = (int)((long)n_cstages * (blockIdx.y + 1) / gridDim.y);
-    plan_walk_level1<KS32, EL>(Cst, s_begin, s_end, smem, nl, xf, xe, P);
+    plan_walk_level1<KS32, EL, FOLD>(Cst, s_begin, s_end, smem, nl, xf, xe, pt);
     __syncthreads();
     for (int i = s_begin + tid; i < s_end; i += 64 * K16_NW) need[(long)blockIdx.x * n_cstages + i] = nl[i - s_begin];
     if (need2_clear != nullptr)
@@ -809,7 +895,7 @@
     exact_list_totals_body<64 * LISTS_WG_TILES>(tile_counts, tiles, blocks_run, groups_run, slots, items, n_items, item_ctr, len_pct, sb, sk, tot_b);
 }
 
-template <int KS32, class EL>
+template <int KS32, class EL, bool FOLD>
 __global__ __launch_bounds__(64 * K16_NW, 3) void exact_plan_fused_kernel(const __bf16* __restrict__ Xb, long N,
                                                                     const char* __restrict__ Cst1, int n_cstages1, const float* __restrict__ cmax2_1,
                                                                     const char* __restrict__ Cst2, int n_slots2, const float* __restrict__ cmax2_2,
@@ -818,7 +904,8 @@
                                                                     const float* __restrict__ wmax2, const float* __restrict__ werr2,
                                                                     ExactBound eb, const int* __restrict__ lastpos, const char* __restrict__ Wst,
                                                                     float* __restrict__ seed_s, int force_all, PlanListsOut lo) {
-    using bf16x8 = typename V8<typename EL::T>::t;
+    using E = typename EL::T;
+    using bf16x8 = typename V8<E>::t;
     constexpr int DP = 32 * KS32;
     constexpr int STAGE = k16_stage_bytes(KS32);
     constexpr int NT = 64 * K16_NW;
@@ -837,14 +924,20 @@
     unsigned long long* nl2 = (unsigned long long*)(smem + 2 * STAGE + (size_t)n_cstages1 * 64 * sizeof(int));
     unsigned long long* nl1 = nl2 + n_cstages2;
     float* p2s = (float*)(nl1 + n_cstages1);
+    E* p2e = (E*)p2s;
 
     bf16x8 xf[K16_SB][KS32];
     bf16x8 xe[K16_SB];
-    float P[K16_SB];
+    PlanTest<EL> pt;
+    float (&P)[K16_SB] = pt.P;
+    E negc2;
     {
         const ExactScales sc1 = ex_scales(xmax2, cmax2_1, cmax2_1 + 1);
         const ExactScales sc2 = ex_scales(xmax2, cmax2_2, cmax2_2 + 1);
         const ExactScales sw = ex_scales(xmax2, wmax2, werr2);
+        const float cf1 = plan_fold_scale<EL>(sc1.sx * sc1.sw * sc1.bmag), cf2 = plan_fold_scale<EL>(sc2.sx * sc2.sw * sc2.bmag);
+        pt.negc = (E)(-cf1);
+        negc2 = (E)(-cf2);
 #pragma unroll
         for (int sb = 0; sb < K16_SB; ++sb) {
             const long row = wave_s0 + sb * 16 + col;
@@ -856,21 +949,33 @@
                 su = plan_row_seed<KS32, EL>(xf[sb], row, q, xer, eb, sw, Wst, lastpos, nullptr, nullptr, seed_s, force_all);
             }
             float bx1, bx2, P2;
-            plan_row_threshold<KS32>(eb, sc1, row < N, q, xer, su, P[sb], bx1);
-            plan_row_threshold<KS32>(eb, sc2, row < N, q, xer, su, P2, bx2);
-            xe[sb] = plan_extra_step<EL>(P[sb] == __builtin_inff() ? bx2 : bx1);
-            if (quad == 0) p2s[wave * (16 * K16_SB) + sb * 16 + col] = P2;
+            plan_row_threshold<KS32, FOLD>(eb, sc1, row < N, q, xer, su, P[sb], bx1);
+            plan_row_threshold<KS32, FOLD>(eb, sc2, row < N, q, xer, su, P2, bx2);
+            xe[sb] = plan_extra_step<EL, FOLD>(P[sb] == __builtin_inff() ? bx2 : bx1, P[sb], cf1);
+            if (quad == 0) {
+                const int at = wave * (16 * K16_SB) + sb * 16 + col;
+                if constexpr (FOLD) {
+                    const PlanParts pp = plan_split_threshold<EL>(P2, cf2);
+                    p2e[4 * at + 1] = (E)pp.p1; p2e[4 * at + 2] = (E)pp.p2; p2e[4 * at + 3] = (E)pp.p3;
+                } else p2s[2 * at] = P2;
+            }
         }
     }
     for (int i = tid; i < n_cstages1 + n_cstages2; i += NT) nl2[i] = 0ull;
 
-    plan_walk_level1<KS32, EL>(Cst1, 0, n_cstages1, smem, nl1, xf, xe, P);
+    plan_walk_level1<KS32, EL, FOLD>(Cst1, 0, n_cstages1, smem, nl1, xf, xe, pt);
     __syncthreads();
     if (wave == 0) plan_level2_list(nl1, n_cstages1, n_slots2, act, &act_n);
 #pragma unroll
-    for (int sb = 0; sb < K16_SB; ++sb) P[sb] = p2s[wave * (16 * K16_SB) + sb * 16 + col];
-    __syncthreads();
-    plan_walk_level2<KS32, EL>(Cst2, act, 0, act_n, smem, nl2, xf, xe, P);
+    for (int sb = 0; sb < K16_SB; ++sb) {
+        const int at = wave * (16 * K16_SB) + sb * 16 + col;
+        if constexpr (FOLD) {
+            if (quad == 0) { xe[sb][1] = p2e[4 * at + 1]; xe[sb][2] = p2e[4 * at + 2]; xe[sb][3] = p2e[4 * at + 3]; }
+        } else P[sb] = p2s[2 * at];
+    }
+    pt.negc = negc2;
+    __syncthreads();
+    plan_walk_level2<KS32, EL, FOLD>(Cst2, act, 0, act_n, smem, nl2, xf, xe, pt);
     __syncthreads();
     if (wave == 0)
         exact_lists_tile<true>(blockIdx.x, lane, nl1, n_cstages1, nl2, lo.n_groups, lo.glist, lo.gcnt, lo.tile_counts, lo.tlist, lo.tcnt, lo.tile_ticket);
diff --git a/xpysom_dask_amd/csrc/somhip.hip b/xpysom_dask_amd/csrc/somhip.hip
--- a/xpysom_dask_amd/csrc/somhip.hip
+++ b/xpysom_dask_amd/csrc/somhip.hip
@@ -165,6 +165,8 @@
         bool fuse_plan = true;
         int hook_plan_parts = 0;
         int64_t plan_fused_launches = 0, plan_split_launches = 0;
+        bool plan_fold = true;
+        int64_t plan_folded = 0, plan_compared = 0;
         DevBuf<int2> items;
         int item_slots = 0;
         int screen_slots = 0;
@@ -1331,6 +1333,7 @@
         if (const char* e = dev_env("SOM_EXACT_CHAIN")) h->ex.chain = std::atoi(e) != 0;
         if (const char* e = dev_env("SOM_EXACT_FUSE_SELECT")) h->ex.fuse_select = std::atoi(e) != 0;
         if (const char* e = dev_env("SOM_EXACT_FUSE_PLAN")) h->ex.fuse_plan = std::atoi(e) != 0;
+        if (const char* e = dev_env("SOM_EXACT_PLAN_FOLD")) h->ex.plan_fold = std::atoi(e) != 0;
         if (const char* e = dev_env("SOM_EXACT_PLAN_PARTS")) h->ex.hook_plan_parts = std::max(0, std::atoi(e));
         if (const char* e = dev_env("SOM_COUNTING_SORT")) h->counting_sort = std::atoi(e) != 0;
         h->use_bands = h->X > 256 || h->Y > 256;
@@ -2300,6 +2303,23 @@
     return 0;
 }
 
+int som_debug_exact_plan_fold_stats(som_handle* h, int64_t* folded, int64_t* compared) {
+    if (!h || !folded || !compared) return fail(h, "som_debug_exact_plan_fold_stats: NULL argument");
+    *folded = h->ex.plan_folded;
+    *compared = h->ex.plan_compared;
+    return 0;
+}
+
+int som_debug_plan_split(int32_t bf16, int64_t n, const float* P, const float* s_bmag, float* out4) {
+    if (n < 0 || (n > 0 && (!P || !s_bmag || !out4))) return 1;
+    for (int64_t i = 0; i < n; ++i) {
+        const float c = bf16 ? plan_fold_scale<Bf16>(s_bmag[i]) : plan_fold_scale<F16>(s_bmag[i]);
+        const PlanParts pp = bf16 ? plan_split_threshold<Bf16>(P[i], c) : plan_split_threshold<F16>(P[i], c);
+        out4[4 * i] = c; out4[4 * i + 1] = pp.p1; out4[4 * i + 2] = pp.p2; out4[4 * i + 3] = pp.p3;
+    }
+    return 0;
+}
+
 int som_debug_exact_last_plan(som_handle* h, int32_t* out8) {
     if (!h || !out8) return fail(h, "som_debug_exact_last_plan: NULL argument");
     const policy::LaunchPlan& p = h->ex.lp;
diff --git a/xpysom_dask_amd/engine.py b/xpysom_dask_amd/engine.py
--- a/xpysom_dask_amd/engine.py
+++ b/xpysom_dask_amd/engine.py
@@ -314,6 +314,11 @@
         self._check(self._lib.som_debug_exact_plan_stats(self._h, C.byref(a), C.byref(b)))
         return a.value, b.value
 
+    def exact_plan_fold_stats(self):
+        a, b = C.c_int64(), C.c_int64()
+        self._check(self._lib.som_debug_exact_plan_fold_stats(self._h, C.byref(a), C.byref(b)))
+        return a.value, b.value
+
     def exact_last_plan(self):
         out = (C.c_int32 * 8)()
         self._check(self._lib.som_debug_exact_last_plan(self._h, out))
```

Result: faster. 551.6 million (median of 6 runs) (+1.1%).
